# janhq/cortex.llamacpp

Measured on AMD Instinct MI355X. Metric: decode tok/s, Llama-3-8B Q4_K_M GGUF (prefill tok/s in `prefill_tok_s`), higher is better.
Workload: dtype int8 dot (Q4_K/Q6_K x Q8_K), f32 accumulate

## Files before the change

cortex.llamacpp_amd/binding.py:

```python
from __future__ import annotations

import ctypes as C
import os

import numpy as np

from .gguf_synth import (BF16, F16, F32, IQ4_NL, IQ4_XS, MXFP4, Q2_K, Q3_K, Q4_0, Q4_1, Q4_K, Q5_0, Q5_1, Q5_K, Q6_K, Q8_0, Q8_K,
                         TQ1_0, TQ2_0)

HERE = os.path.dirname(os.path.abspath(__file__))


class MI355Error(RuntimeError):
    pass


def lib_path() -> str:
    return os.environ.get("MI355_LLAMA_LIB") or os.path.join(HERE, "lib", "libmi355_llama.so")


class ModelParams(C.Structure):
    _fields_ = [("n_gpu_layers", C.c_int32), ("main_gpu", C.c_int32), ("use_mmap", C.c_int32), ("use_mlock", C.c_int32),
                ("tp_rank", C.c_int32), ("tp_size", C.c_int32), ("prefill_planes", C.c_int32)]


class ContextParams(C.Structure):
    _fields_ = [("n_ctx", C.c_uint32), ("n_batch", C.c_uint32), ("n_ubatch", C.c_uint32), ("n_seq_max", C.c_uint32),
                ("type_k", C.c_int32), ("type_v", C.c_int32), ("flash_attn", C.c_int32), ("embeddings", C.c_int32),
                ("use_graphs", C.c_int32), ("logits_to_host", C.c_int32)]


class Batch(C.Structure):
    _fields_ = [("n_tokens", C.c_int32), ("token", C.POINTER(C.c_int32)), ("embd", C.POINTER(C.c_float)),
                ("pos", C.POINTER(C.c_int32)), ("n_seq_id", C.POINTER(C.c_int32)),
                ("seq_id", C.POINTER(C.POINTER(C.c_int32))), ("logits", C.POINTER(C.c_int8))]


class PplStats(C.Structure):
    _fields_ = [("n_chunks", C.c_int64), ("count", C.c_int64), ("top1", C.c_int64), ("dead", C.c_int64), ("same_top", C.c_int64),
                ("has_base", C.c_int32), ("stopped", C.c_int32),
                ("nll", C.c_double), ("nll2", C.c_double), ("nll_base", C.c_double), ("nll2_base", C.c_double), ("kl", C.c_double), ("kl2", C.c_double)]


PPL_CALLBACK = C.CFUNCTYPE(C.c_int32, C.POINTER(PplStats), C.c_void_p)


_vp, _i32, _i64, _u32, _u64, _f32, _sz, _cp = C.c_void_p, C.c_int32, C.c_int64, C.c_uint32, C.c_uint64, C.c_float, C.c_size_t, C.c_char_p
ENGINE_CB = C.CFUNCTYPE(None, C.c_char_p, C.c_char_p, C.c_void_p)
SYMBOLS = {
    "mi355_backend_init": (C.c_int, []),
    "mi355_backend_free": (None, []),
    "mi355_device_count": (C.c_int, []),
    "mi355_last_error": (_cp, []),
    "mi355_time_us": (_i64, []),
    "mi355_print_system_info": (_cp, []),
    "mi355_model_default_params": (ModelParams, []),
    "mi355_model_load_from_file": (_vp, [_cp, ModelParams]),
    "mi355_model_free": (None, [_vp]),
    "mi355_model_n_vocab": (_i32, [_vp]),
    "mi355_model_n_embd": (_i32, [_vp]),
    "mi355_model_n_layer": (_i32, [_vp]),
    "mi355_model_n_head": (_i32, [_vp]),
    "mi355_model_n_head_kv": (_i32, [_vp]),
    "mi355_model_n_ctx_train": (_i32, [_vp]),
    "mi355_model_size": (_u64, [_vp]),
    "mi355_model_cpu_buffer": (_u64, [_vp]),
    "mi355_model_other_buffer": (_u64, [_vp]),
    "mi355_model_bytes_per_token": (_u64, [_vp]),
    "mi355_model_planes_bytes": (_u64, [_vp]),
    "mi355_debug_set_option": (C.c_int, [_cp, _i32]),
    "mi355_model_desc": (_cp, [_vp]),
    "mi355_model_meta_str": (C.c_int, [_vp, _cp, _cp, _sz]),
    "mi355_context_default_params": (ContextParams, []),
    "mi355_context_new": (_vp, [_vp, ContextParams]),
    "mi355_context_free": (None, [_vp]),
    "mi355_n_ctx": (_u32, [_vp]),
    "mi355_n_batch": (_u32, [_vp]),
    "mi355_n_ubatch": (_u32, [_vp]),
    "mi355_context_device_bytes": (_u64, [_vp]),
    "mi355_batch_init": (Batch, [_i32, _i32, _i32]),
    "mi355_batch_free": (None, [Batch]),
    "mi355_decode": (_i32, [_vp, Batch]),
    "mi355_greedy_steps": (_i32, [_vp, _i32, _i32, _i32, _i32, _vp]),
    "mi355_get_logits_ith": (C.POINTER(C.c_float), [_vp, _i32]),
    "mi355_get_argmax_ith": (_i32, [_vp, _i32]),
    "mi355_get_argmax_prob_ith": (_i32, [_vp, _i32, _vp]),
    "mi355_spec_verify": (_i32, [_vp, _i32, _vp, _vp, _vp, _vp]),
    "mi355_get_token_logprobs": (_i32, [_vp, _i32, _vp, _vp, _vp, _vp]),
    "mi355_logits_kl": (_i32, [_vp, _vp, _i32, _vp, _vp, _vp, _vp]),
    "mi355_perplexity": (_i32, [_vp, _vp, _vp, _i64, _i32, _i32, _i32, _vp, _vp, _vp, _vp, _vp]),
    "mi355_imatrix_begin": (_i32, [_vp, _i32]),
    "mi355_imatrix_end": (_i32, [_vp]),
    "mi355_imatrix_clear": (_i32, [_vp]),
    "mi355_imatrix_n_entries": (_i32, [_vp]),
    "mi355_imatrix_entry": (_i32, [_vp, _i32, _vp, _i32, _vp, _vp]),
    "mi355_imatrix_get": (_i32, [_vp, _i32, _vp, _vp]),
    "mi355_speculative_steps": (_i32, [_vp, _vp, _i32, _i32, _i32, _i32, _i32, _i32, _f32, _vp, _vp]),
    "mi355_get_topk_ith": (_i32, [_vp, _i32, _i32, _i32, _vp, _vp, _vp, _f32, _f32, _f32, _vp, _vp]),
    "mi355_debug_mega_steps": (C.c_int64, [_vp]),
    "mi355_debug_engine_steps": (C.c_int64, [_vp]),
    "mi355_debug_fused_skipped_steps": (C.c_int64, [_vp]),
    "mi355_debug_qkv_attn_launches": (C.c_int64, [_vp]),
    "mi355_debug_qkv_attn_plan": (C.c_int64, [C.c_int32] * 10 + [C.POINTER(C.c_int32)]),
    "mi355_set_embeddings": (None, [_vp, _i32]),
    "mi355_get_embeddings_ith": (C.POINTER(C.c_float), [_vp, _i32]),
    "mi355_synchronize": (None, [_vp]),
    "mi355_adapter_lora_init": (_vp, [_vp, _cp]),
    "mi355_adapter_lora_free": (None, [_vp]),
    "mi355_adapter_lora_alpha": (_f32, [_vp]),
    "mi355_adapter_lora_n_pairs": (_i32, [_vp]),
    "mi355_set_adapter_lora": (_i32, [_vp, _vp, _f32]),
    "mi355_rm_adapter_lora": (_i32, [_vp, _vp]),
    "mi355_clear_adapter_lora": (None, [_vp]),
    "mi355_op_lora_delta": (C.c_int, [_i32, _vp, _vp, _vp, _vp, _vp, _vp, _vp, _i64, _i64, _vp, _vp]),
    "mi355_kv_cache_clear": (None, [_vp]),
    "mi355_kv_cache_seq_rm": (_i32, [_vp, _i32, _i32, _i32]),
    "mi355_kv_cache_seq_cp": (None, [_vp, _i32, _i32, _i32, _i32]),
    "mi355_kv_cache_seq_add": (None, [_vp, _i32, _i32, _i32, _i32]),
    "mi355_state_seq_get_size": (_sz, [_vp, _i32]),
    "mi355_state_seq_get_data": (_sz, [_vp, _vp, _sz, _i32]),
    "mi355_state_seq_set_data": (_sz, [_vp, _vp, _sz, _i32]),
    "mi355_state_seq_save_file": (_sz, [_vp, _cp, _i32, _vp, _sz]),
    "mi355_state_seq_load_file": (_sz, [_vp, _cp, _i32, _vp, _sz, C.POINTER(C.c_size_t)]),
    "mi355_debug_state_seq_timing": (None, [_vp, _vp]),
    "mi355_kv_cache_used_cells": (_i32, [_vp]),
    "mi355_debug_enable_taps": (None, [_vp, _i32]),
    "mi355_debug_layer_out": (_i32, [_vp, _i32, _vp, _sz]),
    "mi355_op_quantize_act": (C.c_int, [_i32, _vp, _i64, _i64, _vp]),
    "mi355_op_rms_norm_quant": (C.c_int, [_vp, _vp, _i64, _i64, _f32, _vp, _vp]),
    "mi355_op_swiglu_quant": (C.c_int, [_vp, _vp, _i64, _i64, _vp]),
    "mi355_op_mul_mat": (C.c_int, [_i32, _vp, _i64, _i64, _vp, _i64, _vp, _vp, _vp]),
    "mi355_op_mul_mat_add": (C.c_int, [_i32, _vp, _i64, _i64, _vp, _i64, _vp, _vp]),
    "mi355_op_mul_mat_fused": (C.c_int, [_i32, _vp, _i64, _i64, _vp, _vp, _f32, _vp]),
    "mi355_op_mat_vec_step": (C.c_int, [_i32, _vp, _vp, _vp, _i64, _vp, _i64, _i32, _vp, _i32, _vp, _f32, _i32, _i32, _i32, _vp, _i64, _vp, _vp, _vp]),
    "mi355_op_prompt_mul_mat": (C.c_int, [_i32, _vp, _vp, _vp, _i64, _vp, _i64, _i32, _vp, _i32, _i32, _vp, _f32, _i32, _i64, _vp, _vp]),
    "mi355_op_act_q8k_planes": (C.c_int, [_i32, _vp, _vp, _vp, _f32, _i64, _i64, _vp, _vp, _vp, _vp, _vp, _vp]),
    "mi355_op_f32_to_bf16": (C.c_int, [_vp, _i64, _vp]),
    "mi355_op_mul_mat_bf16": (C.c_int, [_i32, _vp, _vp, _i64, _vp, _i64, _vp, _vp, _i32, _i32, _i32, _i32, _vp]),
    "mi355_op_ffn_gate_up": (C.c_int, [_i32, _vp, _vp, _i64, _i64, _vp, _i64, _vp]),
    "mi355_op_rms_norm_mul": (C.c_int, [_vp, _vp, _i64, _i64, _f32, _vp]),
    "mi355_op_rope": (C.c_int, [_vp, _i32, _i32, _i32, _vp, _i64, _f32, _f32, _vp, _i32]),
    "mi355_op_rope_yarn": (C.c_int, [_vp, _i32, _i32, _i32, _vp, _i64, _f32, _f32, _vp, _i32, _f32, _f32, _f32, _f32]),
    "mi355_op_get_rows": (C.c_int, [_i32, _vp, _i64, _i64, _vp, _i64, _vp]),
    "mi355_op_repack_rows": (C.c_int, [_i32, _vp, _i64, _i64, _vp]),
    "mi355_op_swiglu": (C.c_int, [_vp, _vp, _i64, _vp]),
    "mi355_op_soft_max": (C.c_int, [_vp, _vp, _i64, _i64, _f32, _vp]),
    "mi355_op_moe_route": (C.c_int, [_vp, _i64, _i32, _i32, _vp, _vp]),
    "mi355_op_moe_router": (C.c_int, [_i32, _vp, _i32, _i64, _vp, _i64, _i32, _i32, _vp, _vp, _vp, _vp]),
    "mi355_op_argmax_rows": (C.c_int, [_vp, _i64, _vp, _i32, _i32, _vp]),
    "mi355_op_argmax_prob_rows": (C.c_int, [_vp, _i64, _i32, _vp, _vp]),
    "mi355_op_spec_verify": (C.c_int, [_vp, _i64, _i32, _vp, _i32, _vp, _i32, _vp, _vp, _vp]),
    "mi355_op_token_logprob_rows": (C.c_int, [_vp, _i64, _i32, _vp, _vp, _i32, _vp, _vp]),
    "mi355_op_logits_kl_rows": (C.c_int, [_vp, _i32, _vp, _i32, _i64, _vp, _vp, _i32, _vp, _vp]),
    "mi355_op_imatrix_accum": (C.c_int, [_vp, _vp, _i64, _i64, _i32, _vp, _i32, _vp, _i32, _vp, _vp]),
    "mi355_quantize_chunk": (C.c_int, [_i32, _i32, _vp, _i64, _i64, _vp, _vp]),
    "mi355_quantize_supported": (C.c_int, [_i32]),
    "mi355_quantize_last_times": (C.c_int, [_vp, _vp, _vp]),
    "mi355_op_topk_rows": (C.c_int, [_vp, _i64, _i32, _vp, _i32, _i32, _vp, _vp, _vp, _vp, _vp, _vp, _vp, _vp]),
    "mi355_op_moe_group": (C.c_int, [_vp, _i64, _i32, _i32, _vp, _vp, _vp]),
    "mi355_op_moe_gather_act": (C.c_int, [_vp, _vp, _vp, _vp, _vp, _i64, _i64, _vp, _i64, _vp, _vp, _vp, _vp, _vp]),
    "mi355_op_moe_combine": (C.c_int, [_vp, _vp, _vp, _i64, _i32, _i32, _i32, _vp, _vp]),
    "mi355_op_moe_mul_mat_grouped": (C.c_int, [_i32, _i32, _vp, _vp, _i32, _i64, _i64, _vp, _vp, _i64, _i64, _i64, _vp, _vp]),
    "mi355_op_gather_rows_f32": (C.c_int, [_vp, _i64, _i64, _vp, _i64, _vp]),
    "mi355_op_flash_attn": (C.c_int, [_vp, _i64, _i32, _i32, _i32, _i32, _vp, _i32, _vp, _i32, _vp, _vp, _f32, _vp]),
    "mi355_op_attn_step": (C.c_int, [_vp, _vp, _vp, _i32, _i32, _i32, _i32, _vp, _i32, _vp, _i32, _vp, _i32, _i32, _f32, _i32, _f32, _i32, _vp, _i64, _vp, _i32,
                                     _vp, _vp, _vp, _vp]),
    "mi355_op_attn_decode_neox": (C.c_int, [_vp, _vp, _vp, _i32, _i32, _i32, _i32, _vp, _i32, _vp, _i32, _vp, _i32, _i32, _f32, _f32, _vp, _vp, _f32, _i32,
                                            _vp, _vp, _vp]),
    "mi355_op_flash_attn_seq": (C.c_int, [_vp, _i64, _i32, _i32, _i32, _i32, _vp, _i32, _vp, _i32, _vp, _vp, _vp, _vp, _i32, _f32, _vp]),
    "mi355_op_flash_attn_plan": (C.c_int, [_i64, _i32, _i32, _i32, _i32, _i32, _i32, _vp]),
    "mi355_op_attn_step_seq": (C.c_int, [_vp, _vp, _vp, _i32, _i32, _i32, _i32, _vp, _i32, _vp, _i32, _vp, _vp, _i32, _i32, _i32, _i32, _f32, _i32, _f32, _i32, _vp,
                                         _i64, _vp, _i32, _vp, _vp, _vp, _vp]),
    "mi355_op_attn_decode_neox_seq": (C.c_int, [_vp, _vp, _vp, _i32, _i32, _i32, _i32, _vp, _i32, _vp, _i32, _vp, _vp, _i32, _i32, _i32, _i32, _f32, _f32, _vp, _vp,
                                                _f32, _i32, _vp, _vp, _vp]),
    "mi355_op_attn_batch_step": (C.c_int, [_vp, _vp, _vp, _i64, _i32, _i32, _i32, _i32, _vp, _i32, _vp, _i32, _i32, _vp, _vp, _vp, _vp, _vp, _f32, _i32, _i32, _f32,
                                           _i32, _vp, _vp]),
    "mi355_op_attn_batch_step_planes": (C.c_int, [_vp, _vp, _vp, _i64, _i32, _i32, _i32, _i32, _vp, _i32, _vp, _i32, _i32, _vp, _vp, _vp, _vp, _vp, _f32, _i32, _i32, _f32,
                                           _i32, _vp, _vp, _vp, _vp]),
    "mi355_op_kv_store": (C.c_int, [_i32, _vp, _vp, _vp, _i64, _i32, _i32, _i32, _i32, _i32, _i32, _i32, _i32, _vp, _vp, _f32, _f32, _vp, _vp, _vp, _f32, _vp, _vp]),
    "mi355_op_k_shift": (C.c_int, [_i32, _i32, _i32, _i32, _i32, _i32, _vp, _f32, _f32, _vp, _f32, _f32, _f32, _f32, _vp]),
    "mi355_op_kv_state_pack": (C.c_int, [_i32, _i32, _i32, _i32, _i32, _i32, _vp, _vp, _vp, _i32, _vp]),
    "mi355_op_kv_state_unpack": (C.c_int, [_i32, _i32, _i32, _i32, _i32, _i32, _vp, _vp, _i32, _vp, _vp]),
    "mi355_bench_hbm_read": (C.c_double, [_sz, C.c_int]),
    "mi355_profile_last_decode": (_i32, [_vp, C.POINTER(_cp), C.POINTER(_f32), _i32]),
    "mi355_profile_enable": (None, [_vp, _i32]),
# ... 1021 lines not shown

        def as_dict(s):
            return {name: getattr(s, name) for name, _ in PplStats._fields_}

        raised = []

        def tramp(sp, _user):
            try:
                return 1 if callback(as_dict(sp.contents)) else 0
            except BaseException as ex:
                raised.append(ex)
                return 1

        cb = PPL_CALLBACK(tramp) if callback is not None else None
        r = self.lib.mi355_perplexity(self.h, base.h if base is not None else None, _ptr(tk), tk.size, n_chunk, int(bos), int(seq), _ptr(lp),
                                      _ptr(kl) if kl is not None else None, C.cast(cb, C.c_void_p) if cb is not None else None, None, C.byref(st))
        if raised:
            raise raised[0]
        if r != 0:
            raise MI355Error(f"mi355_perplexity failed: {_err(self.lib)}")
        out = as_dict(st)
        n_scored = int(st.n_chunks) * per
        out["logprobs"] = lp[:n_scored]
        if kl is not None:
            out["kls"] = kl[:n_scored]
        if st.count > 0:
            out["ppl"] = float(np.exp(st.nll / st.count))
            if base is not None:
                out["ppl_base"] = float(np.exp(st.nll_base / st.count))
                out["mean_kl"] = st.kl / st.count
        return out

    def imatrix_begin(self, process_output: bool = False) -> None:
        if self.lib.mi355_imatrix_begin(self.h, int(bool(process_output))) != 0:
            raise MI355Error(f"mi355_imatrix_begin failed: {_err(self.lib)}")

    def imatrix_end(self) -> None:
        if self.lib.mi355_imatrix_end(self.h) != 0:
            raise MI355Error(f"mi355_imatrix_end failed: {_err(self.lib)}")

    def imatrix_clear(self) -> None:
        if self.lib.mi355_imatrix_clear(self.h) != 0:
            raise MI355Error(f"mi355_imatrix_clear failed: {_err(self.lib)}")

    def imatrix_entries(self) -> dict:
        out = {}
        buf = C.create_string_buffer(256)
        for i in range(int(self.lib.mi355_imatrix_n_entries(self.h))):
            ne0, n_mat = C.c_int32(0), C.c_int32(0)
            if self.lib.mi355_imatrix_entry(self.h, i, C.cast(buf, C.c_void_p), 256, C.cast(C.byref(ne0), C.c_void_p), C.cast(C.byref(n_mat), C.c_void_p)) < 0:
                raise MI355Error(f"mi355_imatrix_entry failed: {_err(self.lib)}")
            sum2 = np.zeros((n_mat.value, ne0.value), np.float32)
            counts = np.zeros(n_mat.value, np.int32)
            if self.lib.mi355_imatrix_get(self.h, i, _ptr(sum2), _ptr(counts)) != 0:
                raise MI355Error(f"mi355_imatrix_get failed: {_err(self.lib)}")
            out[buf.value.decode()] = (sum2, counts)
        return out

    def speculative_steps(self, draft_ctx: "Context", first: int, pos0: int, n: int, n_max: int = 16, n_min: int = 0, p_min: float = 0.75, seq: int = 0):
        out = np.empty(n, np.int32); stats = np.zeros(4, np.int64)
        done = self.lib.mi355_speculative_steps(self.h, draft_ctx.h, int(first), int(pos0), int(seq), int(n), int(n_max), int(n_min), float(p_min),
                                                out.ctypes.data, stats.ctypes.data)
        if done != n:
            raise MI355Error(f"mi355_speculative_steps stopped after {done} of {n}: {_err(self.lib)}")
        return out, stats

    def mega_steps(self) -> int:
        return int(self.lib.mi355_debug_mega_steps(self.h))

    def topk(self, k: int, i: int = -1, adj_tok=(), adj_bias=(), adj_count=(), repeat: float = 1.0, freq: float = 0.0, present: float = 0.0):
        at = np.ascontiguousarray(adj_tok, np.int32); ab = np.ascontiguousarray(adj_bias, np.float32); ac = np.ascontiguousarray(adj_count, np.int32)
        toks = np.zeros(k, np.int32); lg = np.zeros(k, np.float32)
        r = self.lib.mi355_get_topk_ith(self.h, i, k, at.size, _ptr(at), _ptr(ab), _ptr(ac), repeat, freq, present, _ptr(toks), _ptr(lg))
        if r != k:
            raise MI355Error(f"mi355_get_topk_ith failed: {_err(self.lib)}")
        return toks, lg

    def fused_skipped_steps(self) -> int:
        return int(self.lib.mi355_debug_fused_skipped_steps(self.h))

    def qkv_attn_launches(self) -> int:
        return int(self.lib.mi355_debug_qkv_attn_launches(self.h))

    def engine_steps(self) -> int:
        return int(self.lib.mi355_debug_engine_steps(self.h))

    def synchronize(self):
        self.lib.mi355_synchronize(self.h)

    def kv_clear(self):
        self.lib.mi355_kv_cache_clear(self.h)

    def kv_seq_rm(self, seq, p0, p1) -> bool:
        return bool(self.lib.mi355_kv_cache_seq_rm(self.h, seq, p0, p1))

    def kv_seq_cp(self, s, d, p0, p1):
        self.lib.mi355_kv_cache_seq_cp(self.h, s, d, p0, p1)

    def kv_seq_add(self, seq, p0, p1, delta):
        self.lib.mi355_kv_cache_seq_add(self.h, seq, p0, p1, delta)

    def state_seq_size(self, seq: int = 0) -> int:
        return int(self.lib.mi355_state_seq_get_size(self.h, int(seq)))

    def state_seq_get(self, seq: int = 0) -> bytes:
        buf = np.zeros(self.state_seq_size(seq), np.uint8)
        n = int(self.lib.mi355_state_seq_get_data(self.h, _ptr(buf), buf.size, int(seq)))
        if n == 0:
            raise MI355Error(f"mi355_state_seq_get_data refused: {_err(self.lib)}")
        return buf[:n].tobytes()

    def state_seq_set(self, seq: int, blob) -> int:
        buf = np.frombuffer(bytes(blob), np.uint8)
        n = int(self.lib.mi355_state_seq_set_data(self.h, buf.ctypes.data if buf.size else None, buf.size, int(seq)))
        if n == 0:
            raise MI355Error(f"mi355_state_seq_set_data refused: {_err(self.lib)}")
        return n

    def state_seq_save_file(self, path: str, seq: int, tokens) -> int:
        tokens = np.ascontiguousarray(tokens, np.int32).reshape(-1)
        n = int(self.lib.mi355_state_seq_save_file(self.h, os.fsencode(path), int(seq), _ptr(tokens), tokens.size))
        if n == 0:
            raise MI355Error(f"mi355_state_seq_save_file refused: {_err(self.lib)}")
        return n

    def state_seq_load_file(self, path: str, seq: int, max_tokens: int = 1 << 20) -> np.ndarray:
        toks = np.zeros(max_tokens, np.int32)
        n_tok = C.c_size_t(0)
        n = int(self.lib.mi355_state_seq_load_file(self.h, os.fsencode(path), int(seq), _ptr(toks), toks.size, C.byref(n_tok)))
        if n == 0:
            raise MI355Error(f"mi355_state_seq_load_file refused: {_err(self.lib)}")
        return toks[:n_tok.value].copy()

    def state_seq_timing(self):
        out = np.zeros(3, np.float32)
        self.lib.mi355_debug_state_seq_timing(self.h, _ptr(out))
        return tuple(float(x) for x in out)

    def kv_used(self) -> int:
        return int(self.lib.mi355_kv_cache_used_cells(self.h))

    def enable_taps(self, on: bool = True):
        self.lib.mi355_debug_enable_taps(self.h, int(on))

    def layer_out(self, il: int, n_tokens: int) -> np.ndarray:
        out = np.zeros((n_tokens, self.model.n_embd), np.float32)
        n = self.lib.mi355_debug_layer_out(self.h, il, _ptr(out), out.size)
        if n < 0:
            raise MI355Error("debug taps not enabled")
        return out[:n]

    def profile(self, on: bool = True):
        self.lib.mi355_profile_enable(self.h, int(on))

    def last_profile(self) -> dict:
        names = (_cp * 64)()
        us = (_f32 * 64)()
        n = self.lib.mi355_profile_last_decode(self.h, names, us, 64)
        return {names[i].decode(): float(us[i]) for i in range(n)}

    def force_moe_ids(self, ids: np.ndarray) -> None:
        ids = np.ascontiguousarray(ids, np.int32)
        rc = self.lib.mi355_debug_force_moe_ids(self.h, _ptr(ids), ids.shape[0], ids.shape[1], ids.shape[2])
        if rc != 0:
            raise MI355Error(f"mi355_debug_force_moe_ids failed ({rc}): {_err(self.lib)}")

# ... 89 lines not shown
```

cortex.llamacpp_amd/csrc/c_api.cc:

```cpp
#include "../../include/mi355_llama.h"

#include <atomic>
#include <memory>
#include <new>
#include <chrono>
#include <cmath>
#include <cstdio>
#include <cstdlib>
#include <cstring>
#include <string>
#include <vector>

#include "../host/clip.h"
#include "../host/engine.h"
#include "../host/hip_backend.h"
#include "../host/log.h"
#include "../host/runtime.h"
#include "../host/attn_chunks.h"
#include "../host/tp_comm.h"
#include "../host/tp_split.h"
#include "../host/vocab.h"

namespace mi355 {
const std::string &last_error_string();
// ... 332 lines not shown
        if (stats) memcpy(stats, st, sizeof st);
        int32_t sid = seq;
        int32_t *sp = &sid;
        int32_t n_seq[SPEC_MAX_DRAFT + 2], pos[SPEC_MAX_DRAFT + 2], toks[SPEC_MAX_DRAFT + 2], ids[SPEC_MAX_DRAFT + 1], draft[SPEC_MAX_DRAFT + 1];
        int32_t *seqs[SPEC_MAX_DRAFT + 2];
        int8_t flags[SPEC_MAX_DRAFT + 2];
        for (int j = 0; j < SPEC_MAX_DRAFT + 2; j++) { n_seq[j] = 1; seqs[j] = sp; }
        auto decode = [&](Context *c, int cnt, bool all_rows) -> bool {
            for (int j = 0; j < cnt; j++) flags[j] = all_rows || j == cnt - 1;
            const int rc = c->decode(cnt, toks, pos, n_seq, seqs, flags);
            if (rc != 0) fail(rc < 0 ? c->last_error : std::string("speculative_steps: no KV cells left for the batch"));
            return rc == 0;
        };
        const int room = (int)std::min(T->cp.n_ctx / T->cp.n_seq_max, D->cp.n_ctx / D->cp.n_seq_max);
        std::vector<int32_t> pend;
        int32_t last = first, p = pos0, dpos = pos0, done = 0;
        while (done < n) {
            const int k_cap = std::max(0, std::min((int)n_max, room - p - 1));
            int k = 0;
            pend.push_back(last);
            if (k_cap > 0) {
                if (pend.size() > (size_t)SPEC_MAX_DRAFT + 2) { fail("speculative_steps: the draft context fell behind"); break; }
                for (size_t j = 0; j < pend.size(); j++) { toks[j] = pend[j]; pos[j] = dpos + (int32_t)j; }
                if (!decode(D, (int)pend.size(), false)) break;
                dpos = p + 1;
                pend.clear();
                bool bad = false;
                for (;;) {
                    float pr = 0.0f;
                    const int32_t t = D->argmax_prob_ith(-1, &pr);
                    if (t < 0) { fail(D->last_error); bad = true; break; }
                    if (pr < p_min) break;
                    draft[k++] = t;
                    if (k == k_cap) break;
                    toks[0] = t; pos[0] = dpos;
                    if (!decode(D, 1, false)) { bad = true; break; }
                    dpos++;
                }
                if (bad) break;
                if (k < n_min) k = 0;
            }
            int a = 0;
            toks[0] = last; pos[0] = p;
            for (int j = 0; j < k; j++) { toks[j + 1] = draft[j]; pos[j + 1] = p + 1 + j; }
            if (!decode(T, k + 1, true)) break;
            if (k > 0) {
                const int32_t gs[2] = {0, k + 1};
                draft[k] = -1;
                if (T->spec_verify(1, gs, draft, ids, &a) < 0) { fail(T->last_error); break; }
            } else {
                ids[0] = T->argmax_ith(0);
                if (ids[0] < 0) { fail(T->last_error.empty() ? "arg-max failed" : T->last_error); break; }
                st[3]++;
            }
            const int m = std::min(a + 1, (int)(n - done));
            st[0]++; st[1] += k; st[2] += m - 1;
            for (int j = 0; j < m; j++) if (out_tokens) out_tokens[done + j] = ids[j];
            done += m;
            const int32_t keep = p + m;
            if (k + 1 > m) T->kv_seq_rm(seq, keep, -1);
            if (dpos > keep) { D->kv_seq_rm(seq, keep, -1); dpos = keep; }
            for (int32_t q = dpos + (int32_t)pend.size(); q < keep; q++) pend.push_back(q == p ? last : ids[q - p - 1]);
            last = ids[m - 1];
            p = keep;
        }
        if (stats) memcpy(stats, st, sizeof st);
        return done;
    )
}
int32_t mi355_get_topk_ith(mi355_context *ctx, int32_t i, int32_t k, int32_t n_adj, const int32_t *adj_tok, const float *adj_bias, const int32_t *adj_count,
                           float penalty_repeat, float penalty_freq, float penalty_present, int32_t *toks_out, float *logits_out) {
    if (!ctx || !toks_out || !logits_out || n_adj < 0 || n_adj > TOPK_MAX_ADJ || (n_adj > 0 && (!adj_tok || !adj_bias || !adj_count))) { fail("bad arguments"); return -1; }
    TopkAdj a{};
    a.n = n_adj; a.repeat = penalty_repeat; a.freq = penalty_freq; a.present = penalty_present;
    for (int j = 0; j < n_adj; j++) { a.tok[j] = adj_tok[j]; a.bias[j] = adj_bias[j]; a.cnt[j] = adj_count[j]; }
    const int r = ctx->c->topk_ith(i, k, a, toks_out, logits_out);
    if (r < 0) fail(ctx->c->last_error.empty() ? "top-k failed" : ctx->c->last_error);
    return r;
}
int64_t mi355_debug_mega_steps(const mi355_context *ctx) { return ctx->c->mega_steps; }
int64_t mi355_debug_engine_steps(const mi355_context *ctx) { return ctx->c->engine_steps; }
int64_t mi355_debug_fused_skipped_steps(const mi355_context *ctx) { return ctx->c->fused_skipped_steps; }
int64_t mi355_debug_qkv_attn_launches(const mi355_context *ctx) { return ctx->c->qkv_attn_launches; }
int64_t mi355_debug_qkv_attn_plan(int32_t type_q, int32_t type_k, int32_t type_v, int32_t type_o, int32_t n_embd, int32_t n_head, int32_t n_head_kv, int32_t head_dim,
                                  int32_t type_kv, int32_t n_kv, int32_t *slots_out) {
    int slots = 0;
    const size_t lds = qkv_attn_out_plan_lds(type_q, type_k, type_v, type_o, n_embd, n_head, n_head_kv, head_dim, type_kv, n_kv, &slots);
    if (slots_out) *slots_out = slots;
    return (int64_t)lds;
}
void mi355_set_embeddings(mi355_context *ctx, int32_t enabled) { ctx->c->embeddings_enabled = enabled != 0 || ctx->c->model->hp.encoder; }
float *mi355_get_embeddings_ith(mi355_context *ctx, int32_t i) { return ctx->c->embeddings_ith(i); }
void mi355_synchronize(mi355_context *ctx) { ctx->c->synchronize(); }

mi355_adapter_lora *mi355_adapter_lora_init(mi355_model *model, const char *path) {
    if (!model || !path) { fail("null model or path"); return nullptr; }
    MI355_GUARD(return nullptr,
        std::string err;
        int status = 0;
        LoraAdapter *a = lora_load(model->m, path, err, status);
        if (!a) { fail(err); return nullptr; }
        mi355_adapter_lora *h = new (std::nothrow) mi355_adapter_lora;
        if (!h) { lora_free(a); fail("out of host memory"); return nullptr; }
        h->a = a;
        return h;
    )
}
void mi355_adapter_lora_free(mi355_adapter_lora *adapter) {
    if (!adapter) return;
    lora_free(adapter->a);
    delete adapter;
}
float mi355_adapter_lora_alpha(const mi355_adapter_lora *adapter) { return adapter ? adapter->a->alpha : 0.0f; }
int32_t mi355_adapter_lora_n_pairs(const mi355_adapter_lora *adapter) { return adapter ? (int32_t)adapter->a->pairs.size() : 0; }
int32_t mi355_set_adapter_lora(mi355_context *ctx, mi355_adapter_lora *adapter, float scale) {
    if (!ctx || !adapter) { fail("null context or adapter"); return MI355_ERR_ARG; }
    MI355_GUARD(return MI355_ERR_ARG,
        if (ctx->c->set_adapter_lora(adapter->a, scale) != 0) { fail(ctx->c->last_error); return MI355_ERR_ARG; }
        return MI355_OK;
    )
}
int32_t mi355_rm_adapter_lora(mi355_context *ctx, mi355_adapter_lora *adapter) {
    if (!ctx || !adapter) { fail("null context or adapter"); return MI355_ERR_ARG; }
    if (ctx->c->rm_adapter_lora(adapter->a) != 0) { fail(ctx->c->last_error); return -1; }
    return MI355_OK;
}
void mi355_clear_adapter_lora(mi355_context *ctx) { if (ctx) ctx->c->clear_adapter_lora(); }

mi355_clip *mi355_clip_model_load(const char *path, int32_t main_gpu) {
    if (!path) { fail("clip_model_load: no path"); return nullptr; }
    MI355_GUARD(return nullptr,
        std::unique_ptr<mi355_clip> c(new mi355_clip);
        const std::string err = c->m.load(path, main_gpu < 0 ? 0 : main_gpu);
        if (!err.empty()) { fail(err); return nullptr; }
        return c.release();
    )
}
void mi355_clip_free(mi355_clip *clip) { delete clip; }
int32_t mi355_clip_n_mmproj_embd(const mi355_clip *clip) { return clip ? clip->m.proj_dim : 0; }
int32_t mi355_clip_n_patches(const mi355_clip *clip) { return clip ? clip->m.n_patches() : 0; }
int32_t mi355_clip_image_size(const mi355_clip *clip) { return clip ? clip->m.image_size : 0; }
int32_t mi355_clip_max_image_rows(const mi355_clip *clip) { return clip ? clip->m.max_image_rows() : 0; }
int32_t mi355_clip_image_preprocess_grid(const mi355_clip *clip, const uint8_t *rgb, int32_t nx, int32_t ny, float *out, size_t out_floats, int32_t *grid_w, int32_t *grid_h) {
    if (!clip || !rgb || !out || nx <= 0 || ny <= 0) { fail("clip_image_preprocess_grid: bad arguments"); return MI355_ERR_ARG; }
    MI355_GUARD(return MI355_ERR_ARG,
        ClipImageU8 img;
        img.nx = nx; img.ny = ny; img.rgb.assign(rgb, rgb + (size_t)3 * nx * ny);
        std::vector<std::vector<float>> imgs;
        int gw = 0, gh = 0;
        clip->m.preprocess_all(img, imgs, gw, gh);
        const size_t per = (size_t)3 * clip->m.image_size * clip->m.image_size;
        if (out_floats < per * imgs.size()) { fail("clip_image_preprocess_grid: output buffer too small"); return MI355_ERR_ARG; }
        for (size_t i = 0; i < imgs.size(); i++) memcpy(out + i * per, imgs[i].data(), per * sizeof(float));
        if (grid_w) *grid_w = gw;
        if (grid_h) *grid_h = gh;
        return (int32_t)imgs.size();
    )
}
int32_t mi355_clip_image_load_from_bytes(const uint8_t *bytes, size_t n_bytes, int32_t *nx, int32_t *ny, uint8_t *rgb_out, size_t rgb_cap) {
    MI355_GUARD(return MI355_ERR_ARG,
        ClipImageU8 img;
        const std::string err = clip_image_load_from_bytes(bytes, n_bytes, img);
        if (!err.empty()) { fail(err); return MI355_ERR_ARG; }
        if (nx) *nx = img.nx;
        if (ny) *ny = img.ny;
        if (rgb_out) {
// ... 1820 lines not shown
    std::vector<KVLayerView> views;
    std::unique_ptr<DevBuf> table, cells, rows;
    size_t row_bytes = 0;
    int init(int type_k, int type_v, int n_layer, int G, int D, int n_cells, const void *const *k_rows, const void *const *v_rows, const int32_t *cell_list, int n, bool distinct) {
        if (!k_rows || !v_rows || !cell_list || n_layer < 1 || n_layer > 1024 || G < 1 || D < 32 || D % 32 || n_cells < 1 || n < 1 || n > n_cells) { fail("kv_state: bad geometry / null argument"); return MI355_ERR_ARG; }
        if ((type_k != T_F16 && type_k != T_Q8_0 && type_k != T_Q4_0) || (type_v != T_F16 && type_v != T_Q8_0 && type_v != T_Q4_0)) { fail("kv_state: bad cache type"); return MI355_ERR_ARG; }
        std::vector<char> seen((size_t)n_cells, 0);
        for (int i = 0; i < n; i++) {
            if (cell_list[i] < 0 || cell_list[i] >= n_cells) { fail("kv_state: cells[" + std::to_string(i) + "] outside the cache"); return MI355_ERR_ARG; }
            if (distinct && seen[(size_t)cell_list[i]]) { fail("kv_state: cells[" + std::to_string(i) + "] listed twice"); return MI355_ERR_ARG; }
            seen[(size_t)cell_list[i]] = 1;
        }
        views.resize((size_t)n_layer);
        for (int il = 0; il < n_layer; il++) {
            if (!k_rows[il] || !v_rows[il]) { fail("kv_state: null layer"); return MI355_ERR_ARG; }
            std::vector<uint8_t> kc, vc;
            std::vector<uint16_t> ks, vs;
            cache_planes_from_rows(type_k, k_rows[il], G, D, n_cells, kc, ks);
            cache_planes_from_rows(type_v, v_rows[il], G, D, n_cells, vc, vs);
            DevBuf *b[4] = {new DevBuf(kc.size()), new DevBuf(ks.size() * 2 + 16), new DevBuf(vc.size()), new DevBuf(vs.size() * 2 + 16)};
            for (DevBuf *p : b) bufs.emplace_back(p);
            if (!b[0]->up(kc.data(), kc.size()) || !b[2]->up(vc.data(), vc.size()) || !b[1]->p || !b[3]->p || (!ks.empty() && !b[1]->up(ks.data(), ks.size() * 2)) ||
                (!vs.empty() && !b[3]->up(vs.data(), vs.size() * 2))) { fail("device alloc/copy failed"); return MI355_ERR_OOM; }
            views[(size_t)il].k = b[0]->as<uint8_t>(); views[(size_t)il].kd = b[1]->as<uint16_t>(); views[(size_t)il].v = b[2]->as<uint8_t>(); views[(size_t)il].vd = b[3]->as<uint16_t>();
        }
        row_bytes = (size_t)n_layer * n * (kv_state_row_bytes(type_k, G, D) + kv_state_row_bytes(type_v, G, D));
        table.reset(new DevBuf(views.size() * sizeof(KVLayerView)));
        cells.reset(new DevBuf((size_t)n * 4));
        rows.reset(new DevBuf(row_bytes));
        if (!table->up(views.data(), views.size() * sizeof(KVLayerView)) || !cells->up(cell_list, (size_t)n * 4) || !rows->p) { fail("device alloc/copy failed"); return MI355_ERR_OOM; }
        return MI355_OK;
    }
};
}

int mi355_op_kv_state_pack(int32_t type_k, int32_t type_v, int32_t n_layer, int32_t G, int32_t D, int32_t n_cells, const void *const *k_rows, const void *const *v_rows,
                           const int32_t *cells, int32_t n, void *out) {
    if (!need_device()) return MI355_ERR_NO_DEVICE;
    if (!out) { fail("kv_state_pack: null output"); return MI355_ERR_ARG; }
    StateOpCache c;
    if (const int rc = c.init(type_k, type_v, n_layer, G, D, n_cells, k_rows, v_rows, cells, n, false)) return rc;
    hipError_t e = launch_kv_state_pack(c.table->as<KVLayerView>(), n_layer, type_k, type_v, G, D, n_cells, c.cells->as<int32_t>(), n, c.rows->as<uint8_t>(), nullptr);
    if (e == hipSuccess) e = hipDeviceSynchronize();
    if (e != hipSuccess) return hip_fail(e, "kv_state_pack");
    return c.rows->down(out, c.row_bytes) ? MI355_OK : MI355_ERR_HIP;
}

int mi355_op_kv_state_unpack(int32_t type_k, int32_t type_v, int32_t n_layer, int32_t G, int32_t D, int32_t n_cells, const void *in, const int32_t *cells, int32_t n,
                             void *const *k_rows, void *const *v_rows) {
    if (!need_device()) return MI355_ERR_NO_DEVICE;
    if (!in) { fail("kv_state_unpack: null input"); return MI355_ERR_ARG; }
    StateOpCache c;
    if (const int rc = c.init(type_k, type_v, n_layer, G, D, n_cells, k_rows, v_rows, cells, n, true)) return rc;
    if (!c.rows->up(in, c.row_bytes)) { fail("device alloc/copy failed"); return MI355_ERR_OOM; }
    hipError_t e = launch_kv_state_unpack(c.table->as<KVLayerView>(), n_layer, type_k, type_v, G, D, n_cells, c.cells->as<int32_t>(), n, c.rows->as<uint8_t>(), nullptr);
    if (e == hipSuccess) e = hipDeviceSynchronize();
    if (e != hipSuccess) return hip_fail(e, "kv_state_unpack");
    for (int il = 0; il < n_layer; il++)
        if (!cache_rows_from_planes(type_k, *c.bufs[(size_t)il * 4], *c.bufs[(size_t)il * 4 + 1], G, D, n_cells, k_rows[il]) ||
            !cache_rows_from_planes(type_v, *c.bufs[(size_t)il * 4 + 2], *c.bufs[(size_t)il * 4 + 3], G, D, n_cells, v_rows[il])) return MI355_ERR_HIP;
    return MI355_OK;
}

int mi355_debug_set_option(const char *name, int32_t value) {
    if (!name) return MI355_ERR_ARG;
    if (!strcmp(name, "mmq_planes")) { g_op_mmq_planes = value != 0; return MI355_OK; }
    if (!strcmp(name, "mmq_tiles")) { mmq_set_tiles(value); return MI355_OK; }
    if (!strcmp(name, "mmq_q80_tiles")) { mmq_q80_set_tiles(value); return MI355_OK; }
    if (!strcmp(name, "mmq_split")) { mmq_set_split(value); return MI355_OK; }
    if (!strcmp(name, "mmq_lds_form")) { mmq_set_lds_form(value); return MI355_OK; }
    if (!strcmp(name, "mmq_ksplit")) { g_op_mmq_ksplit = value != 0; return MI355_OK; }
    if (!strcmp(name, "attn_store_fuse")) { set_attn_store_fuse(value != 0); return MI355_OK; }
    if (!strcmp(name, "rope_fast")) { set_rope_fast(value != 0); return MI355_OK; }
    if (!strcmp(name, "decode_mega") || !strcmp(name, "decode_engine")) {
        if (value > 0 && !experiments_built()) { fail(std::string(name) + ": the experiment kernels are not in this build (MI355_BUILD_EXPERIMENTS=1 python cortex.llamacpp_amd/build.py --force)"); return MI355_ERR_ARG; }
        if (name[7] == 'm') set_decode_mega(value != 0); else set_decode_engine(value);
        return MI355_OK;
    }
    if (!strcmp(name, "tp_p2p")) { tp_p2p_use(value != 0); return MI355_OK; }
    if (!strcmp(name, "tp_p2p_prompt")) { tp_p2p_use_prompt(value != 0); return MI355_OK; }
    if (!strcmp(name, "mmvq_stream")) { mmvq_set_stream(value != 0); return MI355_OK; }
    if (!strcmp(name, "attn_out_fused")) { set_attn_out_fused(value); return MI355_OK; }
    if (!strcmp(name, "qkv_attn_fused")) { set_qkv_attn_fused(value); return MI355_OK; }
    if (!strcmp(name, "moe_group_min")) { set_moe_group_min(value); return MI355_OK; }
    if (!strcmp(name, "moe_q80_grouped")) { set_moe_q80_grouped(value != 0); return MI355_OK; }
    if (!strcmp(name, "fa_v_acc_f16")) { set_fa_v_acc_f16(value); return MI355_OK; }
    if (!strcmp(name, "raise_stream_error")) { debug_raise_stream_error((unsigned)value); return MI355_OK; }
    if (!strcmp(name, "state_stage_kib")) { set_state_stage_max((size_t)(value > 0 ? value : 0) * 1024); return MI355_OK; }
    if (!strcmp(name, "tp_null_group")) { tp_set_null_group(0, value); return MI355_OK; }
    fail(std::string("unknown option ") + name);
    return MI355_ERR_ARG;
}

int mi355_tp_unique_id(void *id_out, size_t cap) {
    if (!need_device()) return MI355_ERR_NO_DEVICE;
    std::string err;
    const int n = tp_unique_id(id_out, cap, err);
    if (n < 0) { fail(err); return MI355_ERR_ARG; }
    return n;
}
int mi355_tp_init(int32_t device, int32_t rank, int32_t size, const void *id, size_t id_len) {
    if (!need_device()) return MI355_ERR_NO_DEVICE;
    if (hipSetDevice(device) != hipSuccess) { fail("hipSetDevice failed"); return MI355_ERR_ARG; }
    std::string err;
    if (tp_init(rank, size, id, id_len, err) != 0) { fail(err); return MI355_ERR_ARG; }
    return MI355_OK;
}
void mi355_tp_shutdown(void) { tp_shutdown(); }
int mi355_tp_worker_main(int sock_fd) {
    try {
        if (!g_backend_ok && mi355_backend_init() != MI355_OK) return 66;
        return tp_split_worker_main(sock_fd);
    } catch (const std::exception &e) {
        fprintf(stderr, "mi355_tp_worker: %s\n", e.what());
        return 70;
    } catch (...) { return 70; }
}
int32_t mi355_tp_rank(void) { return tp_rank(); }
int32_t mi355_tp_size(void) { return tp_size(); }
int mi355_tp_set_host_exchange(mi355_tp_host_exchange fn, void *user, int32_t rank, int32_t size) {
    if (fn && (size < 1 || rank < 0 || rank >= size)) { fail("bad rank / size"); return MI355_ERR_ARG; }
    tp_set_host_exchange(reinterpret_cast<tp_host_exchange_fn>(fn), user, rank, size);
    return MI355_OK;
}

int mi355_tp_p2p_local_handle2(void *out, size_t cap, size_t max_floats, size_t prompt_floats) {
    if (!need_device()) return MI355_ERR_NO_DEVICE;
    std::string err;
    const int n = tp_p2p_local_handle(out, cap, max_floats, prompt_floats, err);
    if (n < 0) { fail(err); return MI355_ERR_ARG; }
    return n;
}
int mi355_tp_p2p_local_handle(void *out, size_t cap, size_t max_floats) { return mi355_tp_p2p_local_handle2(out, cap, max_floats, 0); }
int mi355_tp_p2p_enable(const void *handles, size_t len) {
    if (!need_device()) return MI355_ERR_NO_DEVICE;
    std::string err;
    if (tp_p2p_enable(handles, len, err) != 0) { fail(err); return MI355_ERR_HIP; }
    return MI355_OK;
}
int64_t mi355_tp_p2p_exchanges(void) { return tp_p2p_exchanges(); }
int64_t mi355_tp_p2p_prompt_exchanges(void) { return tp_p2p_prompt_exchanges(); }

double mi355_bench_hbm_read(size_t bytes, int iters) {
    if (!need_device()) return -1.0;
    return hbm_read_probe(bytes, iters);
}

static Vocab *model_vocab(mi355_model *m) {
    if (!m) { fail("null model"); return nullptr; }
    if (!m->vocab_tried) {
        m->vocab_tried = true;
        std::string err;
        m->vocab_ok = m->vocab.load(*m->m->file, err);
        if (!m->vocab_ok) fail("tokenizer: " + err);
    }
    return m->vocab_ok ? &m->vocab : nullptr;
}
int32_t mi355_tokenize(mi355_model *m, const char *text, int32_t text_len, mi355_token *out, int32_t cap, int32_t add_special, int32_t parse_special) {
    MI355_GUARD(return INT32_MIN,
        Vocab *v = model_vocab(m);
        if (!v || !text || text_len < 0) return INT32_MIN;
        const std::vector<int32_t> ids = v->tokenize(std::string(text, (size_t)text_len), add_special != 0, parse_special != 0);
        if ((int64_t)ids.size() > cap || !out) return -(int32_t)ids.size();
        memcpy(out, ids.data(), ids.size() * sizeof(int32_t));
        return (int32_t)ids.size();
    )
// ... 108 lines not shown
```

cortex.llamacpp_amd/host/runtime.cc:

```cpp
#include "runtime.h"

#include <dlfcn.h>
#include "tp_comm.h"
#include "attn_chunks.h"

#include <algorithm>
#include <atomic>
#include <cmath>
#include <cstdarg>
#include <cstdio>
#include <cstring>

namespace mi355 {

unsigned stream_error_epoch();
static unsigned *stream_error_word();

static thread_local std::string g_err;
void set_error(const char *fmt, ...) {
    char buf[1024];
    va_list ap;
    va_start(ap, fmt);
    vsnprintf(buf, sizeof buf, fmt, ap);
    va_end(ap);
// ... 1116 lines not shown
        return launch_mmf16(w.data, (int)w.N, K, x_f32, T, out, ld_out, epi == EPI_ADD ? resid : nullptr, stream_);
    return launch_mmv_float(w.type, w.data, (int)w.N, K, x_f32, T, out, ld_out, epi == EPI_ADD ? resid : nullptr, stream_);
}

static bool bf16_takes_mfma(const DevTensor *const *ws, float *const *outs, int n, int K, int T, int ld_out, const void *xb) {
    bool mfma = true;
    for (int i = 0; i < n; i++) mfma &= mmbf16_applicable(T_BF16, (int)ws[i]->N, K, T, ws[i]->data, xb, outs[i]) && ws[i]->n_expert == 1 && ((n == 1 ? ld_out : (int)ws[i]->N) & 3) == 0;
    return mfma;
}

hipError_t Context::linear_bf16(const DevTensor *const *ws, float *const *outs, const float *const *bias, int n, int K, int T, int ld_out, const float *resid, int epi) {
    if (bf16_takes_mfma(ws, outs, n, K, T, ld_out, xb_)) {
        for (int i = 0; i < n; i++)
            HIP_TRY(launch_mmbf16(ws[i]->data, (int)ws[i]->N, K, xb_, T, outs[i], n == 1 ? ld_out : (int)ws[i]->N, epi == EPI_ADD ? resid : nullptr, bias ? bias[i] : nullptr, 1.0f, false, stream_));
        if (epi == EPI_SWIGLU) HIP_TRY(launch_swiglu(outs[0], outs[1], outs[0], (int64_t)T * ws[0]->N, stream_));
        return hipSuccess;
    }
    MMVBF16Args a{};
    a.n_seg = n; a.K = K; a.epi = epi; a.resid = epi == EPI_ADD ? resid : nullptr; a.xb = xb_;
    for (int i = 0; i < n; i++) a.seg[i] = MMVBF16Seg{ws[i]->data, outs[i], bias ? bias[i] : nullptr, (int)ws[i]->N, n == 1 ? ld_out : (int)ws[i]->N, ws[i]->row_bytes};
    return launch_mmv_bf16_tokens(a, T, stream_);
}

hipError_t Context::linear_multi(const DevTensor *const *ws, float *const *outs, int n, const ActQuant &aq, const float *x_f32, int T, const float *const *bias, bool *bias_done) {
    bool all_q = true, all_bf = n <= 3;
    for (int i = 0; i < n; i++) { all_q &= type_is_quant(ws[i]->type); all_bf &= ws[i]->type == T_BF16 && ws[i]->n_expert == 1; }
    const int K = (int)ws[0]->K;
    if (all_bf) {
        HIP_TRY(launch_f32_to_bf16(x_f32, xb_, (size_t)T * K, stream_));
        HIP_TRY(linear_bf16(ws, outs, bias, n, K, T, 0, nullptr, EPI_STORE));
        if (bias_done) *bias_done = true;
        return hipSuccess;
    }
    const PromptMatmul pm = pending_fuse_.mode == 0 ? prompt_mul_mat_choice(PM_ROLE_MULTI, ws, n, K, T, mmq_ws_) : PromptMatmul();
    if (pm.form == PM_KSPLIT) {
        HIP_TRY(ensure_prep(aq, K, T));
        MMQSeg sg[3];
        for (int i = 0; i < n; i++) sg[i] = MMQSeg{ws[i]->data, ws[i]->row_bytes, (int)ws[i]->N, ws[i]->type, outs[i], (int)ws[i]->N, nullptr, 0};
        return launch_mmq_ksplit_multi(sg, n, K, T, aq, mmq_bh_, mmq_bl_, false, stream_);
    }
    if (pm.form == PM_PLANES) {
        HIP_TRY(ensure_prep(aq, K, T));
        const int nf = pm.n_fused;
        if (nf >= 2) {
            int rows[3], ldo[3], types[3];
            float *o[3];
            for (int i = 0; i < nf; i++) { rows[i] = (int)ws[i]->N; ldo[i] = (int)ws[i]->N; o[i] = outs[i]; types[i] = ws[i]->type; }
            HIP_TRY(launch_mmq_planes_multi(ws[0]->type, ws[0]->planes, rows, o, ldo, nf, K, T, aq, mmq_bh_, mmq_bl_, nullptr, stream_, mmq_ws_, types));
        }
        for (int i = nf; i < n; i++) {
            if (ws[i]->planes) HIP_TRY(launch_mmq_planes(ws[i]->type, ws[i]->planes, (int)ws[i]->N, K, T, aq, mmq_bh_, mmq_bl_, outs[i], (int)ws[i]->N, nullptr, stream_, mmq_ws_));
            else HIP_TRY(launch_mmq(ws[i]->type, ws[i]->data, ws[i]->row_bytes, (int)ws[i]->N, K, T, aq, mmq_bh_, mmq_bl_, outs[i], (int)ws[i]->N, nullptr, stream_));
        }
        return hipSuccess;
    }
    bool any_mmq = false;
    for (int i = 0; i < n; i++) any_mmq |= mmq_applicable(ws[i]->type, K, T) || mmq_q80_applicable(ws[i]->type, K, T) || planes_small(*ws[i], K, T) || q80_copy(*ws[i], K, T);
    if (all_q && n <= 3 && !(any_mmq && pending_fuse_.mode == 0)) {
        MMVQSeg segs[3];
        for (int i = 0; i < n; i++) segs[i] = make_seg(*ws[i], outs[i], (int)ws[i]->N, nullptr, nullptr);
        return mmvq_tokens(segs, n, K, T, EPI_STORE, aq, stream_, pending_fuse_);
    }
    for (int i = 0; i < n; i++) {
        hipError_t e = linear(*ws[i], aq, x_f32, K, T, outs[i], (int)ws[i]->N, nullptr, EPI_STORE);
        if (e != hipSuccess) return e;
    }
    return hipSuccess;
}

static int g_moe_group_min = getenv("MI355_MOE_GROUP_MIN") ? atoi(getenv("MI355_MOE_GROUP_MIN")) : 8;
void set_moe_group_min(int t) { g_moe_group_min = t < 1 ? 1 : t; }
static bool g_moe_q80_grouped = !(getenv("MI355_MOE_Q80_GROUPED") && getenv("MI355_MOE_Q80_GROUPED")[0] == '0');
void set_moe_q80_grouped(bool on) { g_moe_q80_grouped = on; }
static int g_decode_mega = -1;
static bool g_store_fuse = true;
void set_attn_store_fuse(bool on) { g_store_fuse = on; }
static bool store_fuse_enabled() {
    static const bool env_off = getenv("MI355_ATTN_STORE_FUSE") && getenv("MI355_ATTN_STORE_FUSE")[0] == '0';
    return g_store_fuse && !env_off;
}
static bool g_rope_fast = true;
void set_rope_fast(bool on) { g_rope_fast = on; }
void set_decode_mega(bool on) { g_decode_mega = on ? 1 : 0; }

bool Context::mega_prepare() {
    if (mega_state_ != 0) return mega_state_ > 0;
    mega_state_ = -1;
    static const bool mega_env_on = getenv("MI355_MEGA") && getenv("MI355_MEGA")[0] == '1';
    const bool mega_env = g_decode_mega < 0 ? mega_env_on : g_decode_mega > 0;
    const HParams &hp = model->hp;
    const int E = hp.n_embd, FF = hp.n_ff, H = hp.n_head, G = hp.n_head_kv, D = hp.head_dim;
    if (!mega_env || hp.n_expert > 0 || G <= 0 || H % G != 0 || H * D != E) return false;
    const int kb_e = (E + 2047) >> 11, kb_ff = (FF + 2047) >> 11;
    if ((E % 2048) != 0 || (FF % 256) != 0 || !decode_mega_applicable(kb_e, kb_ff, H / G, cp.type_k, cp.type_v, hp.qk_norm)) return false;
    RopeArgs ra = rope_args(*model, false);
    if (ra.neox || (ra.n_rot % 4) != 0 || D != 128 || !kv_store_fast_applicable(G, D, cp.type_k, cp.type_v, ra)) return false;
    std::vector<MegaLayer> ml((size_t)hp.n_layer);
    const int blocks = mega_blocks();
    size_t lds = 0;
    for (int il = 0; il < hp.n_layer; il++) {
        const LayerWeights &L = model->layers[(size_t)il];
        if (!type_is_kq456(L.wq.type) || !type_is_kq456(L.wk.type) || !type_is_kq456(L.wv.type) || !type_is_kq456(L.wo.type) || !type_is_kq456(L.gate.type) || !type_is_kq456(L.up.type) || !type_is_kq456(L.down.type)) return false;
        if (L.gate.type != L.up.type || L.gate.N != L.up.N || L.bq.valid() || L.bk.valid() || L.bv.valid()) return false;
        if ((int)L.wq.K != E || (int)L.wo.K != E || (int)L.gate.K != E || (int)L.down.K != FF) return false;
        MegaLayer &m = ml[(size_t)il];
        m.qkv = single_token_desc(3, E, EPI_STORE, 1, x_, (const float *)L.attn_norm.data, hp.eps, aq_e_);
        m.qkv.seg[0] = make_seg(L.wq, q_, (int)L.wq.N, nullptr, nullptr);
        m.qkv.seg[1] = make_seg(L.wk, k_, (int)L.wk.N, nullptr, nullptr);
        m.qkv.seg[2] = make_seg(L.wv, v_, (int)L.wv.N, nullptr, nullptr);
        m.wo = single_token_desc(1, E, EPI_ADD, 0, nullptr, nullptr, hp.eps, aq_o_);
        m.wo.seg[0] = make_seg(L.wo, x_, E, x_, nullptr);
        m.gate_up = single_token_desc(2, E, EPI_SWIGLU, 1, x_, (const float *)L.ffn_norm.data, hp.eps, aq_e_);
        m.gate_up.seg[0] = make_seg(L.gate, ffn_, FF, nullptr, nullptr);
        m.gate_up.seg[1] = make_seg(L.up, ffn_u_, FF, nullptr, nullptr);
        m.down = single_token_desc(1, FF, EPI_ADD, 2, ffn_, nullptr, hp.eps, aq_ff_);
        m.down.seg[0] = make_seg(L.down, x_, E, x_, nullptr);
        for (MMVQArgs *a : {&m.qkv, &m.wo, &m.gate_up, &m.down}) {
            if (!mmvq_fast_applicable(*a)) return false;
            const size_t l = mmvq_fast_plan(*a, blocks, 4);
            if (!l) return false;
            lds = std::max(lds, l);
        }
        m.kv = kv_[(size_t)il];
    }
    d_mega_layers_ = (MegaLayer *)dalloc(ml.size() * sizeof(MegaLayer));
    if (hipExtMallocWithFlags((void **)&d_mega_sync_, MEGA_SYNC_WORDS * sizeof(unsigned), hipDeviceMallocUncached) != hipSuccess) { d_mega_sync_ = nullptr; return false; }
    allocs_.push_back(d_mega_sync_);
    if (!d_mega_layers_ || !d_mega_sync_) return false;
    if (!h_mega_flag_ && hipHostMalloc((void **)&h_mega_flag_, sizeof(int), hipHostMallocDefault) != hipSuccess) return false;
    *h_mega_flag_ = 0;
    if (hipMemcpy(d_mega_layers_, ml.data(), ml.size() * sizeof(MegaLayer), hipMemcpyHostToDevice) != hipSuccess) return false;
    if (hipMemset(d_mega_sync_, 0, MEGA_SYNC_WORDS * sizeof(unsigned)) != hipSuccess || hipDeviceSynchronize() != hipSuccess) return false;
    if (getenv("MI355_MEGA_PROBE") && getenv("MI355_MEGA_PROBE")[0] == '1')
        d_mega_probe_ = (unsigned long long *)dalloc((size_t)(1 + MEGA_PROBES_PER_LAYER * hp.n_layer) * 8);
    mega_lds_ = lds;
    mega_state_ = 1;
    return true;
}

bool Context::mega_check() {
    if (mega_state_ <= 0 || !h_mega_flag_ || *h_mega_flag_ == 0) return true;
    *h_mega_flag_ = 0;
    (void)hipMemset(d_mega_sync_, 0, MEGA_SYNC_WORDS * sizeof(unsigned));
    (void)hipDeviceSynchronize();
    mega_state_ = -1;
    for (auto &ge : graphs_) (void)hipGraphExecDestroy(ge.second);
    graphs_.clear();
    graph_exec_ = nullptr;
    last_error = "whole-step kernel: device-wide barrier timed out (workgroups not co-resident?); results of the step discarded";
    return false;
}

static int g_decode_engine = -1;
void set_decode_engine(int on) { g_decode_engine = on < 0 ? -1 : on ? 1 : 0; }

static unsigned *stream_error_word() {
    static unsigned *w = [] { unsigned *p = nullptr; if (hipHostMalloc((void **)&p, 64, hipHostMallocDefault) != hipSuccess) p = nullptr; if (p) *p = 0u; return p; }();
    return w;
}

unsigned *install_stream_error_word() {
    unsigned *ew = stream_error_word();
    if (ew) { mmvq_stream_set_error_word(ew); decode_engine_set_error_word(ew); attn_out_set_error_word(ew); tp_p2p_set_error_word(ew); }
    return ew;
}

// ... 91 lines not shown
    if (hipMemcpy(d_engine_layers_, el.data(), el.size() * sizeof(EngineLayer), hipMemcpyHostToDevice) != hipSuccess) return false;
    if (hipMemset(d_engine_gran_, 0, gw * 8) != hipSuccess || hipDeviceSynchronize() != hipSuccess) return false;
    if (const char *pl = getenv("MI355_ENGINE_PROBE")) {
        engine_probe_layer_ = atoi(pl);
        const size_t np = (size_t)num_cu() * 10 * 48;
        d_engine_probe_ = (unsigned long long *)dalloc(np * 8);
        if (d_engine_probe_) (void)hipMemset(d_engine_probe_, 0, np * 8);
        (void)hipDeviceSynchronize();
    }
    engine_state_ = 1;
    return true;
}

hipError_t Context::run_layers_encoder(int T, int n_kv_cap) {
    cur_T_ = T;
    const HParams &hp = model->hp;
    const int E = hp.n_embd, FF = hp.n_ff, H = hp.n_head, G = hp.n_head_kv, D = hp.head_dim;
    RopeArgs ra = rope_args(*model, true);
    const int n_kv_max = std::max(n_kv_cap, 1);
    att_splits_ = flash_attn_pick_splits(T, G, n_kv_max);
    last_layers_mega_ = false; last_layers_engine_ = false;
    HIP_TRY(launch_step_setup_embed(d_pos_, T, ra, rope_cs_, d_cell_pos_, d_cell_seq_, d_cell_, d_seqmask_, nullptr, nullptr, model->tok_embd.type, model->tok_embd.data, E,
                                    d_tok_, x_, stream_));
    if (model->tok_types.valid())
        HIP_TRY(launch_add_qkv_bias(x_, nullptr, nullptr, (const float *)model->tok_types.data, nullptr, nullptr, E, 0, T, stream_));
    HIP_TRY(launch_layer_norm(x_, (const float *)model->tok_norm.data, (const float *)model->tok_norm_b.data, E, T, hp.eps, x_, stream_));
    prof_mark("embed");
    auto quantise_for = [&](const float *x, int K, ActQuant &aq, std::initializer_list<const DevTensor *> ws) -> hipError_t {
        bool k = false, z = false;
        for (const DevTensor *w : ws) if (type_is_quant(w->type)) { if (act_is_q80(w->type)) z = true; else k = true; }
        if (!k && !z) return hipSuccess;
        prep_owner_ = nullptr;
        return launch_quantize(x, K, T, aq, k, z, stream_);
    };
    for (int il = 0; il < hp.n_layer; il++) {
        const LayerWeights &L = model->layers[(size_t)il];
        HIP_TRY(quantise_for(x_, E, aq_e_, {&L.wq, &L.wk, &L.wv}));
        const DevTensor *ws[3] = {&L.wq, &L.wk, &L.wv};
        float *outs[3] = {q_, k_, v_};
        HIP_TRY(linear_multi(ws, outs, 3, aq_e_, x_, T));
        prof_mark("qkv");
        HIP_TRY(launch_rope_kv_store(q_, k_, v_, T, H, G, D, d_pos_, d_cell_, ra, kv_[(size_t)il], cp.type_k, cp.type_v, (int)cp.n_ctx, rope_cs_, stream_));
        prof_mark("rope_kv");
        AttnArgs aa = attn_args(il, T, n_kv_max, d_pos_open_);
        aa.splits = att_splits_;
        aa.pf_splits = flash_attn_prefill_splits(T, H, G, D, n_kv_max);
        while (aa.pf_splits > 1 && flash_attn_workspace_floats(T, H, D, aa.pf_splits) > att_part_floats_) aa.pf_splits >>= 1;
        HIP_TRY(launch_flash_attn(aa, stream_));
        prof_mark("attn");
        HIP_TRY(quantise_for(att_, H * D, aq_o_, {&L.wo}));
        HIP_TRY(linear(L.wo, aq_o_, att_, H * D, T, q_, E, nullptr, EPI_STORE));
        if (L.bo.valid()) HIP_TRY(launch_add_qkv_bias(q_, nullptr, nullptr, (const float *)L.bo.data, nullptr, nullptr, E, 0, T, stream_));
        HIP_TRY(launch_add(q_, x_, xn_, (int64_t)T * E, stream_));
        HIP_TRY(launch_layer_norm(xn_, (const float *)L.attn_out_norm.data, (const float *)L.attn_out_norm_b.data, E, T, hp.eps, xn_, stream_));
        prof_mark("attn_out");
        HIP_TRY(quantise_for(xn_, E, aq_e_, {&L.gate, &L.up}));
        HIP_TRY(linear(L.gate, aq_e_, xn_, E, T, ffn_, FF, nullptr, EPI_STORE));
        HIP_TRY(linear(L.up, aq_e_, xn_, E, T, ffn_u_, FF, nullptr, EPI_STORE));
        HIP_TRY(launch_swiglu(ffn_, ffn_u_, ffn_, (int64_t)T * FF, stream_));
        prof_mark("ffn_gate_up");
        HIP_TRY(quantise_for(ffn_, FF, aq_ff_, {&L.down}));
        HIP_TRY(linear(L.down, aq_ff_, ffn_, FF, T, q_, E, nullptr, EPI_STORE));
        HIP_TRY(launch_add(q_, xn_, x_, (int64_t)T * E, stream_));
        HIP_TRY(launch_layer_norm(x_, (const float *)L.layer_out_norm.data, (const float *)L.layer_out_norm_b.data, E, T, hp.eps, x_, stream_));
        prof_mark("ffn_down");
        if (debug_taps_ && dbg_) HIP_TRY(hipMemcpyAsync(dbg_ + (size_t)il * cp.n_ubatch * E, x_, (size_t)T * E * 4, hipMemcpyDeviceToDevice, stream_));
    }
    return hipSuccess;
}


Context::Step Context::step_constants(int T, int n_kv_cap) const {
    static const int attn_mode = getenv("MI355_ATTN_MODE") ? atoi(getenv("MI355_ATTN_MODE")) : 2;
    static const bool rope_fast_env = !(getenv("MI355_ROPE_FAST") && getenv("MI355_ROPE_FAST")[0] == '0');
    static const bool fuse_down_env = !(getenv("MI355_FUSE_DOWN") && getenv("MI355_FUSE_DOWN")[0] == '0');
    const HParams &hp = model->hp;
    Step st;
    st.T = T;
    st.n_kv_max = std::max(n_kv_cap, 1);
    st.ra_step = rope_args(*model, true);
    st.tp = hp.tp_exchange;
    st.chunk_lists = chunk_lmax_ > 0;
    st.attn_mode = attn_mode; st.rope_fast = rope_fast_env && g_rope_fast; st.fuse_down_env = fuse_down_env;
    st.out = st.tp ? tp_part_ : x_;
    st.resid = !st.tp || hp.tp_rank == 0 ? x_ : nullptr;
    return st;
}

AttnArgs Context::attn_args(int il, int T, int n_kv_max, const int32_t *tok_pos) const {
    const HParams &hp = model->hp;
    AttnArgs aa{};
    aa.q = q_; aa.out = att_; aa.kv = kv_[(size_t)il]; aa.type_k = cp.type_k; aa.type_v = cp.type_v;
    aa.T = T; aa.H = hp.n_head; aa.G = hp.n_head_kv; aa.D = hp.head_dim; aa.n_ctx = (int)cp.n_ctx;
    aa.cell_pos = d_cell_pos_; aa.cell_seq = d_cell_seq_; aa.tok_pos = tok_pos; aa.tok_seq = d_seq_;
    aa.n_kv_dev = d_nkv_; aa.n_kv_max = n_kv_max; aa.scale = 1.0f / sqrtf((float)hp.head_dim); aa.part = att_part_;
    return aa;
}
void Context::attn_chunk_lists(AttnArgs &aa) const {
    aa.tok_chunks = d_chunks_; aa.tok_nchunks = d_chunks_ + (size_t)64 * chunk_stride_; aa.chunk_stride = chunk_stride_;
    aa.splits = std::max(chunk_cap_, chunk_lmax_);
}

Context::AttnPlan Context::plan_attn(int il, const Step &st) const {
    const HParams &hp = model->hp;
    const LayerWeights &L = model->layers[(size_t)il];
    const int E = hp.n_embd, T = st.T;
    AttnPlan p{};
    p.ra = layer_rope(st.ra_step, L, hp.eps);
    p.qkv_float = !type_is_quant(L.wq.type) || !type_is_quant(L.wk.type) || !type_is_quant(L.wv.type);
    p.qkv_lora = f32_rows(il, LORA_Q) || f32_rows(il, LORA_K) || f32_rows(il, LORA_V);
    p.qkv_prologue = !p.qkv_float && can_fuse(E, T) && !p.qkv_lora;
    AttnArgs &aa = p.aa;
    aa = attn_args(il, T, st.n_kv_max, d_pos_);
    const bool o_q = type_is_quant(L.wo.type);
    aa.out_q = o_q ? &aq_o_ : nullptr; aa.out_q8k = !act_is_q80(L.wo.type); aa.out_q80 = act_is_q80(L.wo.type);
    p.o_planes = o_q && aa.out_q8k && T >= 3;
    if (p.o_planes) { aa.out_bh = mmq_bh_; aa.out_bl = mmq_bl_; }
    const bool v16 = fa_v_acc_f16_enabled() && cp.type_k == T_F16 && cp.type_v == T_F16;
    p.decode_attn = !v16 && flash_attn_decode_applicable(aa, p.ra);
    if (p.decode_attn) {
        aa.splits = flash_attn_decode_splits(st.n_kv_max);
        if (st.chunk_lists) attn_chunk_lists(aa);
        p.fused_step = st.attn_mode > 0 && flash_attn_decode_fused_applicable(aa, p.ra);
    }
    p.ao_seg = make_seg(L.wo, st.out, E, st.resid, nullptr);
    p.ao_epi = st.resid ? EPI_ADD : EPI_STORE;
    p.af = aa;
    if (p.decode_attn && p.fused_step && st.attn_mode == 2 && !st.engine && il < 255 && !attn_out_off_ && !attn_out_skip_step_ && !(st.tp && tp_uses_host()) && !f32_rows(il, LORA_O)) {
        p.af.splits = attn_out_fused_splits(p.af);
        if (st.chunk_lists) p.af.splits = aa.splits;
        p.ao_form = attn_out_fused_applicable(p.af, p.ra, p.ao_seg, (int)L.wo.K, p.ao_epi);
    }
    if (p.ao_form && p.qkv_prologue && !st.tp && d_qkv_gran_ && !(L.bq.valid() || L.bk.valid() || L.bv.valid())) {
        QKVFuse &qf = p.qf;
        qf.seg[0] = make_seg(L.wq, q_, (int)L.wq.N, nullptr, nullptr);
        qf.seg[1] = make_seg(L.wk, k_, (int)L.wk.N, nullptr, nullptr);
        qf.seg[2] = make_seg(L.wv, v_, (int)L.wv.N, nullptr, nullptr);
        qf.nx = x_; qf.nw = (const float *)L.attn_norm.data; qf.neps = hp.eps; qf.K = E; qf.gran = d_qkv_gran_;
        p.qkv_in_attn = qkv_attn_out_applicable(p.af, p.ra, p.ao_seg, (int)L.wo.K, p.ao_epi, qf);
    }
    return p;
}

hipError_t Context::attn_qkv(int il, const Step &st, const AttnPlan &p) {
    const HParams &hp = model->hp;
    const LayerWeights &L = model->layers[(size_t)il];
    const int E = hp.n_embd, T = st.T;
    if (p.qkv_in_attn) return hipSuccess;
    if (st.engine && il > 0) return hipSuccess;
    if (p.qkv_prologue) {
        pending_fuse_.mode = 1; pending_fuse_.x = x_; pending_fuse_.w = (const float *)L.attn_norm.data; pending_fuse_.eps = hp.eps;
    } else {
        const bool need_k = (type_is_quant(L.wq.type) && !act_is_q80(L.wq.type)) || (type_is_quant(L.wk.type) && !act_is_q80(L.wk.type)) || (type_is_quant(L.wv.type) && !act_is_q80(L.wv.type));
        const bool need_0 = act_is_q80(L.wq.type) || act_is_q80(L.wk.type) || act_is_q80(L.wv.type);
        const bool pl = need_k && T >= 3;
        HIP_TRY(launch_rmsnorm_quant(x_, (const float *)L.attn_norm.data, E, T, hp.eps, p.qkv_float || p.qkv_lora ? xn_ : nullptr, &aq_e_, need_k, need_0, stream_,
                                     pl ? mmq_bh_ : nullptr, pl ? mmq_bl_ : nullptr));
        prep_owner_ = nullptr;
        if (pl) prep_written(aq_e_, E, T);
        prof_mark("norm_quant");
        if (imx_on_) HIP_TRY(imx_collect(il, IMX_QKV, xn_, nullptr, E, T, nullptr, nullptr));
    }
    const DevTensor *ws[3] = {&L.wq, &L.wk, &L.wv};
    float *outs[3] = {q_, k_, v_};
    const float *bias[3] = {L.bq.valid() ? (const float *)L.bq.data : nullptr, L.bk.valid() ? (const float *)L.bk.data : nullptr, L.bv.valid() ? (const float *)L.bv.data : nullptr};
    bool bias_done = false;
    HIP_TRY(linear_multi(ws, outs, 3, aq_e_, xn_, T, bias, &bias_done));
    pending_fuse_ = Fuse();
    if (p.qkv_lora) {
        const int targets[3] = {LORA_Q, LORA_K, LORA_V}, lds[3] = {(int)L.wq.N, (int)L.wk.N, (int)L.wv.N};
        HIP_TRY(lora_add(il, targets, outs, lds, 3, xn_, E, E, T));
    }
    if (!bias_done && (bias[0] || bias[1] || bias[2]))
        HIP_TRY(launch_add_qkv_bias(q_, k_, v_, bias[0], bias[1], bias[2], hp.n_head * hp.head_dim, hp.n_head_kv * hp.head_dim, T, stream_));
    prof_mark("qkv");
    return hipSuccess;
}

hipError_t Context::attn_core(int il, const Step &st, const AttnPlan &p) {
    const HParams &hp = model->hp;
    const LayerWeights &L = model->layers[(size_t)il];
    const int H = hp.n_head, G = hp.n_head_kv, D = hp.head_dim, T = st.T;
    const KVLayerView &kv = kv_[(size_t)il];
    unsigned *ao_flags = d_ao_flags_ + (size_t)il * 64 * ATT_SYNC_STRIDE;
    if (p.qkv_in_attn) {
        HIP_TRY(launch_qkv_attn_out(p.af, rope_cs_, p.ra, d_cell_, att_counters_, ao_flags, d_ao_gran_, il, d_step_serial_, p.ao_seg, (int)L.wo.K, p.ao_epi, p.qf, stream_));
        qkv_attn_launches++;
        prof_mark("qkv");
    } else if (p.fused_step) {
        if (p.ao_form)
            HIP_TRY(launch_attn_out_fused(p.af, rope_cs_, p.ra, k_, v_, d_cell_, att_counters_, ao_flags, d_ao_gran_, il, d_step_serial_, p.ao_seg, (int)L.wo.K, p.ao_epi, stream_));
        else
            HIP_TRY(launch_flash_attn_decode_fused(p.aa, rope_cs_, p.ra, k_, v_, d_cell_, st.attn_mode == 2 ? att_counters_ : nullptr, stream_));
    } else if (p.decode_attn && batch_distinct_ && store_fuse_enabled()) {
        HIP_TRY(launch_flash_attn_decode(p.aa, rope_cs_, p.ra, stream_, k_, v_, d_cell_));
    } else if (p.decode_attn && kv_store_fast_applicable(G, D, cp.type_k, cp.type_v, p.ra)) {
        HIP_TRY(launch_kv_store_fast(k_, v_, T, G, D, rope_cs_, p.ra, d_cell_, kv, cp.type_k, cp.type_v, (int)cp.n_ctx, stream_));
        prof_mark("rope_kv");
        HIP_TRY(launch_flash_attn_decode(p.aa, rope_cs_, p.ra, stream_));
    } else {
        if (st.rope_fast && rope_cs_ && rope_q_kv_store_fast_applicable(H, G, D, cp.type_k, cp.type_v, p.ra))
            HIP_TRY(launch_rope_q_kv_store_fast(q_, k_, v_, T, H, G, D, rope_cs_, p.ra, d_cell_, kv, cp.type_k, cp.type_v, (int)cp.n_ctx, stream_));
        else
            HIP_TRY(launch_rope_kv_store(q_, k_, v_, T, H, G, D, d_pos_, d_cell_, p.ra, kv, cp.type_k, cp.type_v, (int)cp.n_ctx, rope_cs_, stream_));
        prof_mark("rope_kv");
        AttnArgs aa = p.aa;
        aa.splits = att_splits_;
        aa.pf_splits = flash_attn_prefill_splits(T, H, G, D, std::min(st.n_kv_max, cur_max_pos_ + 1));
        while (aa.pf_splits > 1 && flash_attn_workspace_floats(T, H, D, aa.pf_splits) > att_part_floats_) aa.pf_splits >>= 1;
        HIP_TRY(launch_flash_attn(aa, stream_));
    }
    prof_mark("attn");
    if (p.o_planes) prep_written(aq_o_, (int)L.wo.K, T);
    else if (prep_owner_ == aq_o_.qs) prep_owner_ = nullptr;
    return hipSuccess;
}

hipError_t Context::attn_output(int il, const Step &st, const AttnPlan &p) {
    const LayerWeights &L = model->layers[(size_t)il];
    if (p.ao_form) return hipSuccess;
    HIP_TRY(linear(L.wo, aq_o_, att_, (int)L.wo.K, st.T, st.out, model->hp.n_embd, st.resid, p.ao_epi));
    if (imx_on_) HIP_TRY(imx_collect(il, IMX_O, att_, nullptr, (int)L.wo.K, st.T, nullptr, nullptr));
    if (lora_on(il, LORA_O)) {
        const int target = LORA_O, ld = model->hp.n_embd;
        float *out = st.out;
        HIP_TRY(lora_add(il, &target, &out, &ld, 1, att_, (int)L.wo.K, (int)L.wo.K, st.T));
    }
    return hipSuccess;
}

hipError_t Context::quantise_for_down(int il, int T, bool combined, bool planes_any_T) {
    const int FF = model->hp.n_ff;
    const bool k = !act_is_q80(model->layers[(size_t)il].down.type), pl = k && (planes_any_T || T >= 3);
    int8_t *bh = pl ? mmq_bh_ : nullptr, *bl = pl ? mmq_bl_ : nullptr;
    if (combined) HIP_TRY(launch_quantize(ffn_, FF, T, aq_ff_, k, !k, stream_, bh, bl));
    else HIP_TRY(launch_swiglu_quant(ffn_, ffn_u_, FF, T, aq_ff_, k, !k, stream_, bh, bl));
    prep_owner_ = nullptr;
    if (pl) prep_written(aq_ff_, FF, T);
    return hipSuccess;
}

hipError_t Context::ffn_dense_gate_up(int il, const Step &st, bool &quantised) {
    const HParams &hp = model->hp;
    const LayerWeights &L = model->layers[(size_t)il];
    const int E = hp.n_embd, FF = hp.n_ff, T = st.T;
    quantised = false;
    const bool gq = type_is_quant(L.gate.type), uq = type_is_quant(L.up.type);
    const bool fk = (gq && !act_is_q80(L.gate.type)) || (uq && !act_is_q80(L.up.type));
    const bool f0 = act_is_q80(L.gate.type) || act_is_q80(L.up.type);
    const bool lora_gu = f32_rows(il, LORA_GATE) || f32_rows(il, LORA_UP), lora_any = lora_gu || f32_rows(il, LORA_DOWN);
    const bool fuse_ffn = gq && uq && L.gate.type == L.up.type && can_fuse(E, T) && !lora_any;
    Fuse fz;
    if (fuse_ffn) {
        fz.mode = 1; fz.x = x_; fz.w = (const float *)L.ffn_norm.data; fz.eps = hp.eps;
    } else {
        const bool pl = fk && T >= 3;
        HIP_TRY(launch_rmsnorm_quant(x_, (const float *)L.ffn_norm.data, E, T, hp.eps, (!gq || !uq || lora_gu) ? xn_ : nullptr, &aq_e_, fk, f0, stream_,
                                     pl ? mmq_bh_ : nullptr, pl ? mmq_bl_ : nullptr));
        prep_owner_ = nullptr;
        if (pl) prep_written(aq_e_, E, T);
        prof_mark("norm_quant");
        if (imx_on_) HIP_TRY(imx_collect(il, IMX_FFN_IN, xn_, nullptr, E, T, nullptr, nullptr));
    }
    const bool down_q = type_is_quant(L.down.type) && (FF % 32) == 0;
    const bool ffn_mmq = (mmq_q80_applicable(L.gate.type, E, T) && mmq_q80_applicable(L.up.type, E, T)) ||
                         (mmq_applicable(L.gate.type, E, T) && mmq_applicable(L.up.type, E, T)) ||
                         (mmq_ksplit_applicable(L.gate.type, E, T) && mmq_ksplit_applicable(L.up.type, E, T)) ||
                         (planes_small(L.gate, E, T) && planes_small(L.up, E, T)) || (q80_copy(L.gate, E, T) && q80_copy(L.up, E, T));
    const DevTensor *gu_w[2] = {&L.gate, &L.up};
    const PromptMatmul gu_pm = fuse_ffn ? PromptMatmul() : prompt_mul_mat_choice(PM_ROLE_GATE_UP, gu_w, 2, E, T, mmq_ws_);
    const bool ffn_ks = gu_pm.form == PM_KSPLIT;
    if (lora_any) {
        HIP_TRY(linear(L.gate, aq_e_, xn_, E, T, ffn_, FF, nullptr, EPI_STORE));
        HIP_TRY(linear(L.up, aq_e_, xn_, E, T, ffn_u_, FF, nullptr, EPI_STORE));
        if (lora_gu) {
            const int targets[2] = {LORA_GATE, LORA_UP}, lds[2] = {FF, FF};
            float *outs[2] = {ffn_, ffn_u_};
            HIP_TRY(lora_add(il, targets, outs, lds, 2, xn_, E, E, T));
        }
        quantised = T > 1 && down_q && !f32_rows(il, LORA_DOWN);
        if (quantised) HIP_TRY(quantise_for_down(il, T, false, false));
        else HIP_TRY(launch_swiglu(ffn_, ffn_u_, ffn_, (int64_t)T * FF, stream_));
        if (imx_on_) HIP_TRY(imx_collect(il, IMX_FFN_DOWN, ffn_, nullptr, FF, T, nullptr, nullptr));
    } else if (gq && uq && L.gate.type == L.up.type && !ffn_mmq) {
        MMVQSeg segs[2] = {make_seg(L.gate, ffn_, FF, nullptr, nullptr), make_seg(L.up, ffn_u_, FF, nullptr, nullptr)};
        HIP_TRY(mmvq_tokens(segs, 2, E, T, EPI_SWIGLU, aq_e_, stream_, fz));
    } else if (L.gate.type == T_BF16 && L.up.type == T_BF16 && L.gate.N == L.up.N) {
        const DevTensor *gu[2] = {&L.gate, &L.up};
        float *go[2] = {ffn_, ffn_u_};
        HIP_TRY(launch_f32_to_bf16(xn_, xb_, (size_t)T * E, stream_));
        quantised = T > 1 && down_q && bf16_takes_mfma(gu, go, 2, E, T, 0, xb_);
        HIP_TRY(linear_bf16(gu, go, nullptr, 2, E, T, 0, nullptr, quantised ? EPI_STORE : EPI_SWIGLU));
        if (quantised) HIP_TRY(quantise_for_down(il, T, false, false));
    } else if (ffn_ks) {
        if (gu_pm.need_prep) HIP_TRY(ensure_prep(aq_e_, E, T));
        MMQSeg sg[2] = {{L.gate.data, L.gate.row_bytes, (int)L.gate.N, L.gate.type, ffn_, FF, nullptr, 0},
                        {L.up.data, L.up.row_bytes, (int)L.up.N, L.up.type, ffn_u_, FF, nullptr, 0}};
        const bool pair = gu_pm.swiglu;
        HIP_TRY(launch_mmq_ksplit_multi(sg, 2, E, T, aq_e_, mmq_bh_, mmq_bl_, pair, stream_));
        quantised = !pair && down_q;
        if (quantised) HIP_TRY(quantise_for_down(il, T, false, true));
        else if (!pair) HIP_TRY(launch_swiglu(ffn_, ffn_u_, ffn_, (int64_t)T * FF, stream_));
    } else if (T > 1 && gu_pm.form == PM_PLANES) {
        HIP_TRY(launch_mmq_planes_swiglu(L.gate.type, L.gate.planes, L.up.planes, (int)L.gate.N, E, T, aq_e_, ffn_, FF, stream_));
        quantised = down_q;
        if (quantised) HIP_TRY(quantise_for_down(il, T, true, false));
    } else {
        HIP_TRY(linear(L.gate, aq_e_, xn_, E, T, ffn_, FF, nullptr, EPI_STORE));
        HIP_TRY(linear(L.up, aq_e_, xn_, E, T, ffn_u_, FF, nullptr, EPI_STORE));
        quantised = T > 1 && down_q;
        if (quantised) HIP_TRY(quantise_for_down(il, T, false, false));
        else HIP_TRY(launch_swiglu(ffn_, ffn_u_, ffn_, (int64_t)T * FF, stream_));
    }
    prof_mark("ffn_gate_up");
    return hipSuccess;
}

hipError_t Context::ffn_down(int il, const Step &st, bool quantised, int *n_matvec) {
    const HParams &hp = model->hp;
    const LayerWeights &L = model->layers[(size_t)il];
    const int E = hp.n_embd, FF = hp.n_ff, T = st.T;
    const int epi = st.resid ? EPI_ADD : EPI_STORE;
    const bool lora_down = f32_rows(il, LORA_DOWN);
    const bool fuse_down = !lora_down && st.fuse_down_env && T == 1 && type_is_quant(L.down.type) &&
                           (((FF % 256) == 0 && mmvq_fast_kb_ok((FF + 2047) / 2048)) || ((FF % 256) != 0 && (FF % 32) == 0 && FF <= 8192 && act_is_q80(L.down.type)));
    if (fuse_down && !st.tp && L.down_lo.valid() && L.down_hi.valid()) {
        const int Kh = (int)L.down_lo.K;
        pending_fuse_.mode = 2; pending_fuse_.x = ffn_;
        HIP_TRY(linear(L.down_lo, aq_ff_, ffn_, Kh, T, st.out, E, st.resid, epi));
        pending_fuse_.mode = 2; pending_fuse_.x = ffn_ + Kh;
        HIP_TRY(linear(L.down_hi, aq_ff_, ffn_ + Kh, Kh, T, st.out, E, st.out, EPI_ADD));
        pending_fuse_ = Fuse();
        if (n_matvec) *n_matvec = 2;
        return hipSuccess;
    }
    if (n_matvec) *n_matvec = 1;
    if (fuse_down) {
        pending_fuse_.mode = 2; pending_fuse_.x = ffn_;
    } else if (type_is_quant(L.down.type) && !quantised) {
        HIP_TRY(launch_quantize(ffn_, FF, T, aq_ff_, !act_is_q80(L.down.type), act_is_q80(L.down.type), stream_));
        prep_owner_ = nullptr;
        prof_mark("quant");
    }
    HIP_TRY(linear(L.down, aq_ff_, ffn_, FF, T, st.out, E, st.resid, epi));
    pending_fuse_ = Fuse();
    if (lora_down) {
        const int target = LORA_DOWN;
        float *out = st.out;
        HIP_TRY(lora_add(il, &target, &out, &E, 1, ffn_, FF, FF, T));
    }
    return hipSuccess;
}

bool Context::moe_selected_desc(int il, MMVQArgs &a, MMVQArgs &d) const {
    const HParams &hp = model->hp;
    const LayerWeights &L = model->layers[(size_t)il];
    const int E = hp.n_embd, FF = hp.n_ff, KU = hp.n_expert_used;
    if (KU < 2 || KU > 8 || (int)cp.n_ubatch < KU || L.gate_exps.type != L.up_exps.type) return false;
    const bool prologue = can_fuse(E, 1) && !act_is_q80(L.gate_exps.type);
    a = single_token_desc(2, E, EPI_SWIGLU, prologue ? 1 : 0, prologue ? x_ : nullptr, prologue ? (const float *)L.ffn_norm.data : nullptr, prologue ? hp.eps : 0.0f, aq_e_);
    a.n_sel = KU; a.sel_out_stride = FF;
    a.seg[0] = make_seg(L.gate_exps, ffn_, FF, nullptr, moe_ids_);
    a.seg[1] = make_seg(L.up_exps, ffn_u_, FF, nullptr, moe_ids_);
    d = single_token_desc(1, FF, EPI_STORE, 2, ffn_, nullptr, 0.0f, aq_ff_);
    d.n_sel = KU; d.sel_nx_stride = FF; d.sel_out_stride = E;
    d.seg[0] = make_seg(L.down_exps, moe_out_, E, nullptr, moe_ids_);
    return mmvq_fast_applicable(a) && mmvq_fast_applicable(d);
}

hipError_t Context::moe_grouped_one_launch(int il, int T) {
    const HParams &hp = model->hp;
    const LayerWeights &L = model->layers[(size_t)il];
    const int E = hp.n_embd, FF = hp.n_ff, KU = hp.n_expert_used, NE = hp.n_expert, GR = T * KU;
    HIP_TRY(launch_moe_gather_act(aq_e_, moe_tok_, GR, E, aq_eg_, stream_));
    prep_owner_ = nullptr;
    const size_t ps_gu = L.gate_exps.planes_bytes / (size_t)L.gate_exps.n_expert, ps_d = L.down_exps.planes_bytes / (size_t)L.down_exps.n_expert;
    HIP_TRY(launch_mmq_planes_swiglu_moe(L.gate_exps.type, L.gate_exps.planes, L.up_exps.planes, ps_gu, NE, moe_meta_, (int)L.gate_exps.N, E, GR, aq_eg_, ffn_g_, FF, stream_));
    if (imx_on_) HIP_TRY(imx_collect(il, IMX_FFN_DOWN, ffn_g_, nullptr, FF, GR, nullptr, moe_meta_));
    HIP_TRY(launch_quantize(ffn_g_, FF, GR, aq_ffg_, true, false, stream_));
    HIP_TRY(launch_mmq_planes_moe(L.down_exps.type, L.down_exps.planes, ps_d, NE, moe_meta_, (int)L.down_exps.N, FF, GR, aq_ffg_, y_g_, E, stream_));
    return launch_moe_scatter_combine(x_, y_g_, moe_w_, moe_slot_, T, E, KU, stream_);
}

hipError_t Context::moe_grouped_q80(int il, int T) {
    const HParams &hp = model->hp;
    const LayerWeights &L = model->layers[(size_t)il];
    const int E = hp.n_embd, FF = hp.n_ff, KU = hp.n_expert_used, NE = hp.n_expert, GR = T * KU;
    HIP_TRY(launch_moe_gather_act(aq_e_, moe_tok_, GR, E, aq_eg_, stream_));
    prep_owner_ = nullptr;
    const uint8_t *w_gu[2] = {L.gate_exps.planes, L.up_exps.planes}, *w_d[1] = {L.down_exps.planes};
    float *o_gu[2] = {ffn_g_, ffn_ug_}, *o_d[1] = {y_g_};
    HIP_TRY(launch_mmq_q80_moe(L.gate_exps.type, w_gu, o_gu, 2, L.gate_exps.planes_bytes / (size_t)L.gate_exps.n_expert, NE, moe_meta_, (int)L.gate_exps.N, E, GR, aq_eg_, FF, stream_));
    if (imx_on_) HIP_TRY(imx_collect(il, IMX_FFN_DOWN, ffn_g_, ffn_ug_, FF, GR, nullptr, moe_meta_));
    HIP_TRY(launch_swiglu_quant(ffn_g_, ffn_ug_, FF, GR, aq_ffg_, false, true, stream_, nullptr, nullptr));
    HIP_TRY(launch_mmq_q80_moe(L.down_exps.type, w_d, o_d, 1, L.down_exps.planes_bytes / (size_t)L.down_exps.n_expert, NE, moe_meta_, (int)L.down_exps.N, FF, GR, aq_ffg_, E, stream_));
    return launch_moe_scatter_combine(x_, y_g_, moe_w_, moe_slot_, T, E, KU, stream_);
}

hipError_t Context::moe_grouped_per_expert(int il, int T, bool q80_any) {
    const HParams &hp = model->hp;
    const LayerWeights &L = model->layers[(size_t)il];
    const int E = hp.n_embd, FF = hp.n_ff, KU = hp.n_expert_used, NE = hp.n_expert, GR = T * KU;
    HIP_TRY(hipMemcpyAsync(h_moe_meta_, moe_meta_, (size_t)(2 * NE + 1) * 4, hipMemcpyDeviceToHost, stream_));
    HIP_TRY(launch_moe_gather_act(aq_e_, moe_tok_, GR, E, aq_eg_, stream_));
    prep_owner_ = nullptr;
    HIP_TRY(hipStreamSynchronize(stream_));
    auto view = [](const DevTensor &w, int e) {
        DevTensor v = w;
        v.data = w.data + (size_t)e * w.row_bytes * (size_t)w.N;
        v.n_expert = 1;
        v.planes = w.planes ? w.planes + (size_t)e * (w.planes_bytes / (size_t)w.n_expert) : nullptr;
        return v;
    };
    auto rows = [](const ActQuant &q, int r0, int K) {
        ActQuant v;
        if (q.qs) { v.qs = q.qs + (size_t)r0 * K; v.d = q.d + (size_t)r0 * (K / 256); v.bsums = q.bsums + (size_t)r0 * (K / 16); }
        if (q.qs0) { v.qs0 = q.qs0 + (size_t)r0 * K; v.d0 = q.d0 + (size_t)r0 * (K / 32); }
        return v;
    };
    auto copy_batch = [&](const DevTensor &w, int e, const ActQuant &q, int K, int n_e, float *out, int ld_out) {
        return launch_mmq_q80(w.planes + (size_t)e * (w.planes_bytes / (size_t)w.n_expert), mmq_q80_copy_row_bytes(w.type, K), (int)w.N, K, n_e, q, out, ld_out, nullptr, stream_,
                              mmq_q80_copy_form(w.type), true);
    };
    const bool pl_gu = !act_is_q80(L.gate_exps.type) || !act_is_q80(L.up_exps.type), pl_d = !act_is_q80(L.down_exps.type);
    if (pl_gu) HIP_TRY(launch_mmq_prep(aq_eg_, E, GR, mmq_bh_, mmq_bl_, stream_));
    hipError_t e_exp = hipSuccess;
    for (int e = 0; e < NE && e_exp == hipSuccess; e++) {
        const int n_e = h_moe_meta_[e], r0 = h_moe_meta_[NE + e];
        if (n_e <= 0) continue;
        if (pl_gu) { bh_over_ = mmq_bh_ + (size_t)r0 * (E >> 4); bl_over_ = mmq_bl_ + (size_t)r0 * (E >> 4); }
        if (q80_any) {
            e_exp = copy_batch(L.gate_exps, e, rows(aq_eg_, r0, E), E, n_e, ffn_g_ + (size_t)r0 * FF, FF);
            if (e_exp == hipSuccess) e_exp = copy_batch(L.up_exps, e, rows(aq_eg_, r0, E), E, n_e, ffn_ug_ + (size_t)r0 * FF, FF);
            continue;
        }
        e_exp = linear(view(L.gate_exps, e), rows(aq_eg_, r0, E), nullptr, E, n_e, ffn_g_ + (size_t)r0 * FF, FF, nullptr, EPI_STORE);
        if (e_exp == hipSuccess) e_exp = linear(view(L.up_exps, e), rows(aq_eg_, r0, E), nullptr, E, n_e, ffn_ug_ + (size_t)r0 * FF, FF, nullptr, EPI_STORE);
    }
    bh_over_ = bl_over_ = nullptr;
    HIP_TRY(e_exp);
    if (imx_on_) HIP_TRY(imx_collect(il, IMX_FFN_DOWN, ffn_g_, ffn_ug_, FF, GR, nullptr, moe_meta_));
    HIP_TRY(launch_swiglu_quant(ffn_g_, ffn_ug_, FF, GR, aq_ffg_, !act_is_q80(L.down_exps.type), act_is_q80(L.down_exps.type), stream_,
                                pl_d ? mmq_bh_ : nullptr, pl_d ? mmq_bl_ : nullptr));
    prep_owner_ = nullptr;
    for (int e = 0; e < NE && e_exp == hipSuccess; e++) {
        const int n_e = h_moe_meta_[e], r0 = h_moe_meta_[NE + e];
        if (n_e <= 0) continue;
        if (pl_d) { bh_over_ = mmq_bh_ + (size_t)r0 * (FF >> 4); bl_over_ = mmq_bl_ + (size_t)r0 * (FF >> 4); }
        if (q80_any) { e_exp = copy_batch(L.down_exps, e, rows(aq_ffg_, r0, FF), FF, n_e, y_g_ + (size_t)r0 * E, E); continue; }
        e_exp = linear(view(L.down_exps, e), rows(aq_ffg_, r0, FF), nullptr, FF, n_e, y_g_ + (size_t)r0 * E, E, nullptr, EPI_STORE);
    }
    bh_over_ = bl_over_ = nullptr;
    HIP_TRY(e_exp);
    return launch_moe_scatter_combine(x_, y_g_, moe_w_, moe_slot_, T, E, KU, stream_);
}

hipError_t Context::moe_selected(int il, int T) {
    const HParams &hp = model->hp;
    const LayerWeights &L = model->layers[(size_t)il];
    const int E = hp.n_embd, FF = hp.n_ff, KU = hp.n_expert_used;
    MMVQArgs a{}, d{};
    if (T == 1 && moe_selected_desc(il, a, d)) {
        HIP_TRY(launch_mmvq(a, stream_));
        HIP_TRY(launch_mmvq(d, stream_));
        return launch_moe_combine(x_, moe_out_, moe_w_, T, E, KU, (size_t)T * E, stream_);
    }
    const bool fuse_q = type_is_kq456(L.down_exps.type) && (FF % 256) == 0 && mmvq_fast_kb_ok((FF + 2047) / 2048);
    for (int t = 0; t < T; t++) {
        for (int j = 0; j < KU; j++) {
            const int32_t *esel = moe_ids_ + (size_t)t * KU + j;
            a = MMVQArgs{};
            a.n_seg = 2; a.K = E; a.T = 1; a.epi = EPI_SWIGLU;
            a.seg[0] = make_seg(L.gate_exps, ffn_ + (size_t)t * FF, FF, nullptr, esel);
            a.seg[1] = make_seg(L.up_exps, ffn_u_ + (size_t)t * FF, FF, nullptr, esel);
            chunk_act(a, aq_e_, E, t);
            if (L.gate_exps.type == L.up_exps.type) {
                HIP_TRY(launch_mmvq(a, stream_));
            } else {
                a.epi = EPI_STORE;
                HIP_TRY(launch_mmvq(a, stream_));
                HIP_TRY(launch_swiglu(ffn_ + (size_t)t * FF, ffn_u_ + (size_t)t * FF, ffn_ + (size_t)t * FF, FF, stream_));
            }
            if (!fuse_q) { HIP_TRY(launch_quantize(ffn_ + (size_t)t * FF, FF, 1, aq_ff_, !act_is_q80(L.down_exps.type), act_is_q80(L.down_exps.type), stream_)); prep_owner_ = nullptr; }
            d = MMVQArgs{};
            d.n_seg = 1; d.K = FF; d.T = 1; d.epi = EPI_STORE;
            if (fuse_q) { d.fuse_mode = 2; d.nx = ffn_ + (size_t)t * FF; }
            d.seg[0] = make_seg(L.down_exps, moe_out_ + ((size_t)j * T + t) * E, E, nullptr, esel);
            chunk_act(d, aq_ff_, FF, 0);
            HIP_TRY(launch_mmvq(d, stream_));
        }
    }
    return launch_moe_combine(x_, moe_out_, moe_w_, T, E, KU, (size_t)T * E, stream_);
}

hipError_t Context::ffn_moe(int il, const Step &st) {
    const HParams &hp = model->hp;
    const LayerWeights &L = model->layers[(size_t)il];
    const int E = hp.n_embd, FF = hp.n_ff, T = st.T, KU = hp.n_expert_used;
    HIP_TRY(launch_rmsnorm_quant(x_, (const float *)L.ffn_norm.data, E, T, hp.eps, xn_, &aq_e_,
                                 !act_is_q80(L.gate_exps.type) || !act_is_q80(L.up_exps.type), act_is_q80(L.gate_exps.type) || act_is_q80(L.up_exps.type), stream_));
    prep_owner_ = nullptr;
    prof_mark("norm_quant");
    const int32_t *forced = moe_forced_T_ == T ? d_moe_forced_ + (size_t)il * T * KU : nullptr;
    if ((L.gate_inp.type == T_F32 || L.gate_inp.type == T_F16) && hp.n_expert <= 8) {
        HIP_TRY(launch_moe_router(L.gate_inp.type, L.gate_inp.data, hp.n_expert, E, xn_, T, KU, router_, moe_ids_, moe_w_, stream_, forced));
    } else {
        HIP_TRY(launch_mmv_float(L.gate_inp.type, L.gate_inp.data, hp.n_expert, E, xn_, T, router_, hp.n_expert, nullptr, stream_));
        HIP_TRY(launch_moe_route(router_, T, hp.n_expert, KU, moe_ids_, moe_w_, stream_, forced));
    }
    prof_mark("moe_route");
    const bool exps_q = type_is_quant(L.gate_exps.type) && type_is_quant(L.up_exps.type) && type_is_quant(L.down_exps.type);
    if (imx_on_) HIP_TRY(imx_collect(il, IMX_ROUTER, xn_, nullptr, E, T, nullptr, nullptr));
    if (exps_q && (T >= g_moe_group_min || imx_on_) && aq_eg_.qs) {
        HIP_TRY(launch_moe_group(moe_ids_, T, KU, hp.n_expert, moe_meta_, moe_slot_, moe_tok_, stream_));
        if (imx_on_) HIP_TRY(imx_collect(il, IMX_FFN_IN, xn_, nullptr, E, T * KU, moe_tok_, moe_meta_));
        const bool one_launch = T >= 32 && L.gate_exps.planes && L.up_exps.planes && L.down_exps.planes && L.gate_exps.type == L.up_exps.type &&
                                L.gate_exps.N == L.up_exps.N && mmq_planes_moe_ok(L.gate_exps.type, (int)L.gate_exps.N, E) &&
                                mmq_planes_moe_ok(L.down_exps.type, (int)L.down_exps.N, FF) && (L.gate_exps.N % 64) == 0;
        const bool q80_ok = T >= 32 && L.gate_exps.planes && L.up_exps.planes && L.down_exps.planes && L.gate_exps.type == T_MXFP4 && L.up_exps.type == T_MXFP4 &&
                            L.down_exps.type == T_MXFP4 && L.gate_exps.N == L.up_exps.N && mmq_q80_moe_ok(T_MXFP4, (int)L.gate_exps.N, E) &&
                            mmq_q80_moe_ok(T_MXFP4, (int)L.down_exps.N, FF) && aq_eg_.qs0 && aq_ffg_.qs0;
        if (q80_ok && g_moe_q80_grouped) HIP_TRY(moe_grouped_q80(il, T));
        else HIP_TRY(one_launch ? moe_grouped_one_launch(il, T) : moe_grouped_per_expert(il, T, q80_ok));
    } else {
        HIP_TRY(moe_selected(il, T));
    }
    prof_mark("moe_ffn");
    return hipSuccess;
}

hipError_t Context::ffn_block(int il, const Step &st) {
    if (model->hp.n_expert > 0) return ffn_moe(il, st);
    bool quantised = false;
    HIP_TRY(ffn_dense_gate_up(il, st, quantised));
    HIP_TRY(ffn_down(il, st, quantised));
    if (st.tp) HIP_TRY(tp_reduce_into_x(st.T));
    prof_mark("ffn_down");
    return hipSuccess;
}

hipError_t Context::tap_layer(int il, int T) {
    if (!debug_taps_ || !dbg_) return hipSuccess;
    return hipMemcpyAsync(dbg_ + (size_t)il * cp.n_ubatch * model->hp.n_embd, x_, (size_t)T * model->hp.n_embd * 4, hipMemcpyDeviceToDevice, stream_);
}

hipError_t Context::run_layers(int T, int n_kv_cap) {
    if (model->hp.encoder) return run_layers_encoder(T, n_kv_cap);
    cur_T_ = T;
    const HParams &hp = model->hp;
    const int E = hp.n_embd, FF = hp.n_ff;
    Step st = step_constants(T, n_kv_cap);
    att_splits_ = flash_attn_pick_splits(T, hp.n_head_kv, st.n_kv_max);

    bool mega = T == 1 && !profile_ && !debug_taps_ && !ub_embd_ && lora_.empty() && !imx_on_ && mega_prepare();
    AttnArgs ma{};
    if (mega) {
        ma = attn_args(0, 1, st.n_kv_max, d_pos_);
        ma.out_q = &aq_o_; ma.out_q8k = !act_is_q80(model->layers[0].wo.type); ma.out_q80 = false;
        ma.splits = flash_attn_decode_splits(st.n_kv_max);
        if (st.chunk_lists) attn_chunk_lists(ma);
        mega = flash_attn_decode_fused_applicable(ma, st.ra_step);
    }
    st.engine = T == 1 && !mega && !profile_ && !debug_taps_ && !ub_embd_ && lora_.empty() && !imx_on_ && engine_prepare();
    last_layers_engine_ = st.engine;
    HIP_TRY(launch_step_setup_embed(d_pos_, T, st.ra_step, rope_cs_, d_cell_pos_, d_cell_seq_, d_cell_, d_seqmask_, mega ? d_mega_sync_ : nullptr,
                                    d_step_serial_, model->tok_embd.type, model->tok_embd.data, E, d_tok_, x_, stream_));
    if (ub_embd_) HIP_TRY(hipMemcpyAsync(x_, ub_embd_, (size_t)T * E * sizeof(float), hipMemcpyHostToDevice, stream_));
    prof_mark("embed");
    last_layers_mega_ = mega;
    if (mega)
        return launch_decode_mega(d_mega_layers_, hp.n_layer, (E + 2047) >> 11, (FF + 2047) >> 11, ma, rope_cs_, st.ra_step.n_rot, k_, v_, d_cell_,
                                  att_counters_, d_mega_sync_, h_mega_flag_, d_mega_probe_, mega_lds_, stream_);

    for (int il = 0; il < hp.n_layer; il++) {
        const AttnPlan ap = plan_attn(il, st);
        HIP_TRY(attn_qkv(il, st, ap));
        HIP_TRY(attn_core(il, st, ap));
        if (st.engine) {
            HIP_TRY(launch_decode_engine(d_engine_layers_ + il, E, FF, d_engine_gran_, d_engine_epoch_, il, il == engine_probe_layer_ ? d_engine_probe_ : nullptr, stream_));
        } else {
            HIP_TRY(attn_output(il, st, ap));
            if (st.tp) HIP_TRY(tp_reduce_into_x(T));
            prof_mark("attn_out");
            HIP_TRY(ffn_block(il, st));
        }
        HIP_TRY(tap_layer(il, T));
    }
    return hipSuccess;
}

hipError_t Context::tp_reduce_into_x(int T) {
    return tp_all_reduce_sum(tp_part_, x_, (size_t)T * model->hp.n_embd, stream_);
}

hipError_t Context::run_output(int n_out, int out_base) {
    logits_on_host_ = false;
    if (n_out <= 0) return hipSuccess;
    const HParams &hp = model->hp;
    const int E = hp.n_embd, V = hp.n_vocab;
    float *const xo = cur_T_ == 1 && n_out == 1 ? x_ : xo_;
    if (xo != x_) HIP_TRY(launch_gather_rows_f32(x_, d_outrow_, n_out, E, xo_, stream_));
    if (hp.encoder) {
        HIP_TRY(hipMemcpyAsync(d_embd_ + (size_t)out_base * E, xo, (size_t)n_out * E * 4, hipMemcpyDeviceToDevice, stream_));
        prof_mark("embd");
        return hipSuccess;
    }
    if (embeddings_enabled) {
        HIP_TRY(launch_rmsnorm_quant(xo, (const float *)model->out_norm.data, E, n_out, hp.eps, d_embd_ + (size_t)out_base * E, nullptr, false, false, stream_));
        prof_mark("embd");
        return hipSuccess;
    }
    const bool oq = type_is_quant(model->output.type);
    const bool imx_head = imx_on_ && imx_output_;
    const bool lora_head = lora_on(-1, LORA_OUTPUT);
    const bool head_rows = lora_head || imx_head;
    static const bool zc_env = !(getenv("MI355_LOGITS_ZERO_COPY") && getenv("MI355_LOGITS_ZERO_COPY")[0] == '0');
    logits_on_host_ = zc_env && oq && cur_T_ == 1 && n_out == 1 && cp.logits_to_host && !hp.tp_exchange && h_logits_ != nullptr && !head_rows;
    if (oq && can_fuse(E, n_out) && !head_rows) {
        pending_fuse_.mode = 1; pending_fuse_.x = xo; pending_fuse_.w = (const float *)model->out_norm.data; pending_fuse_.eps = hp.eps;
    } else {
        prep_owner_ = nullptr;
        HIP_TRY(launch_rmsnorm_quant(xo, (const float *)model->out_norm.data, E, n_out, hp.eps, oq && !head_rows ? nullptr : xn_, &aq_e_,
                                     oq && !act_is_q80(model->output.type), act_is_q80(model->output.type), stream_));
        prof_mark("norm_quant");
        if (imx_head) HIP_TRY(imx_collect(-1, IMX_QKV, xn_, nullptr, E, n_out, nullptr, nullptr));
    }
    float *lg = d_logits_ + (size_t)out_base * V;
    const int VL = hp.n_vocab_local, P = hp.tp_size;
    if (hp.tp_exchange && VL * P == V) {
        if (n_out > 1 && (size_t)n_out > tp_logits_rows_) {
            HIP_TRY(hipStreamSynchronize(stream_));
            tp_logits_ = (float *)dalloc((size_t)n_out * V * 4);
            if (!tp_logits_) return hipErrorOutOfMemory;
            tp_logits_rows_ = (size_t)n_out;
            HIP_TRY(hipDeviceSynchronize());
        }
        float *gathered = n_out == 1 ? lg : tp_logits_;
        float *part = gathered + (size_t)hp.tp_rank * n_out * VL;
        HIP_TRY(linear(model->output, aq_e_, xn_, E, n_out, part, VL, nullptr, EPI_STORE));
        pending_fuse_ = Fuse();
        HIP_TRY(tp_all_gather(part, gathered, (size_t)n_out * VL, stream_));
        for (int r = 0; r < P && n_out > 1; r++)
            HIP_TRY(hipMemcpy2DAsync(lg + (size_t)r * VL, (size_t)V * 4, tp_logits_ + (size_t)r * n_out * VL, (size_t)VL * 4, (size_t)VL * 4, (size_t)n_out,
                                     hipMemcpyDeviceToDevice, stream_));
    } else {
        if (logits_on_host_) pending_fuse_.out_host = h_logits_ + (size_t)out_base * V;
        HIP_TRY(linear(model->output, aq_e_, xn_, E, n_out, lg, V, nullptr, EPI_STORE));
        if (lora_head) {
            const int target = LORA_OUTPUT;
            HIP_TRY(lora_add(-1, &target, &lg, &V, 1, xn_, E, E, n_out));
        }
    }
    pending_fuse_ = Fuse();
    prof_mark("lm_head");
    for (int r0 = 0; r0 < n_out; r0 += (int)cp.n_ubatch) {
        const int nr = std::min((int)cp.n_ubatch, n_out - r0);
        HIP_TRY(launch_argmax_rows(lg + (size_t)r0 * V, V, nr, h_argmax_ + out_base + r0, argmax_scratch_, (int)cp.n_ubatch, stream_));
    }
    prof_mark("argmax");
    return hipSuccess;
}

int Context::decode_ubatch(int n, const int32_t *tokens, const int32_t *pos, const int32_t *seq, const uint64_t *seqmask,
                           const int8_t *flags, int out_base) {
    { const unsigned long long ls = next_launch_serial(); if (!first_unchecked_launch_) first_unchecked_launch_ = ls; }
    cur_max_pos_ = 0;
    for (int i = 0; i < n; i++) cur_max_pos_ = std::max(cur_max_pos_, (int)pos[i]);
    std::vector<int> tcell;
    if (!alloc_cells(n, seqmask, tcell)) return 1;
    for (int i = 0; i < n; i++) {
        KVCell &c = cells_[(size_t)tcell[(size_t)i]];
        c.pos = pos[i]; c.seqs = seqmask[i]; c.delta = 0;
    }
    int hi = 0;
    for (int i = (int)cells_.size() - 1; i >= 0; i--) if (cells_[(size_t)i].pos >= 0) { hi = i + 1; break; }
    n_kv_ = std::min((int)cp.n_ctx, (hi + 31) & ~31);

    if (meta_dirty_) {
        std::vector<int32_t> cpos(cells_.size());
        std::vector<uint64_t> cseq(cells_.size());
        for (size_t i = 0; i < cells_.size(); i++) { cpos[i] = cells_[i].pos; cseq[i] = cells_[i].seqs; }
        if (hipMemcpyAsync(d_cell_pos_, cpos.data(), cpos.size() * 4, hipMemcpyHostToDevice, stream_) != hipSuccess ||
            hipMemcpyAsync(d_cell_seq_, cseq.data(), cseq.size() * 8, hipMemcpyHostToDevice, stream_) != hipSuccess ||
            hipStreamSynchronize(stream_) != hipSuccess) { last_error = "cell table upload failed"; return -1; }
        meta_dirty_ = false;
    }
    if (stage_event_) (void)hipEventSynchronize(stage_event_);
    const size_t T = ((size_t)cp.n_ubatch + 1) & ~(size_t)1;
    int32_t *h_nkv = (int32_t *)h_stage_;
    int32_t *h_tok = (int32_t *)(h_stage_ + 16), *h_pos = h_tok + T, *h_seq = h_pos + T, *h_cell = h_seq + T, *h_out = h_cell + T;
    uint64_t *h_mask = (uint64_t *)(h_out + T);
    h_nkv[0] = n_kv_;
    int n_out = 0;
    for (int i = 0; i < n; i++) {
        h_tok[i] = tokens[i]; h_pos[i] = pos[i]; h_seq[i] = seq[i]; h_cell[i] = tcell[(size_t)i]; h_mask[i] = seqmask[i];
        if (flags[i]) h_out[n_out++] = i;
    }
    if (hipMemcpyAsync(d_stage_, h_stage_, stage_bytes_, hipMemcpyHostToDevice, stream_) != hipSuccess) { last_error = "token upload failed"; return -1; }
    chunk_lmax_ = 0;
    batch_distinct_ = n >= 2 && n <= 64;
    {
        uint64_t seen = 0;
        for (int i = 0; i < n && batch_distinct_; i++) {
            const uint64_t mk = seqmask[i];
            if (mk == 0 || (mk & (mk - 1)) != 0 || (seen & mk) != 0) batch_distinct_ = false;
            seen |= mk;
        }
    }
    bool lists_usable = false;
    {
        const HParams &hp = model->hp;
        RopeArgs ra = rope_args(*model, false);
        AttnArgs aa{};
        aa.T = n; aa.H = hp.n_head; aa.G = hp.n_head_kv; aa.D = hp.head_dim; aa.n_kv_max = n_kv_; aa.type_k = cp.type_k; aa.type_v = cp.type_v;
        lists_usable = n <= 64 && flash_attn_decode_applicable(aa, ra) && kv_store_fast_applicable(aa.G, aa.D, cp.type_k, cp.type_v, ra);
    }
    if ((n >= 2 || cp.n_seq_max > 1) && lists_usable) {
        chunk_lmax_ = build_attn_chunk_lists(n_kv_, (int)cells_.size(), [&](int i, int32_t &p, uint64_t &m) { p = cells_[(size_t)i].pos; m = cells_[(size_t)i].seqs; },
                                             seq, n, chunk_stride_, h_chunks_, h_chunks_ + (size_t)64 * chunk_stride_);
        if (hipMemcpyAsync(d_chunks_, h_chunks_, (size_t)64 * (chunk_stride_ + 1) * 4, hipMemcpyHostToDevice, stream_) != hipSuccess) { last_error = "chunk list upload failed"; return -1; }
    }
    static const bool profiler_safe = getenv("MI355_PROFILER_SAFE") && getenv("MI355_PROFILER_SAFE")[0] == '1';
    if (profiler_safe) (void)hipStreamSynchronize(stream_);
    if (!stage_event_) (void)hipEventCreateWithFlags(&stage_event_, hipEventDisableTiming);
    if (stage_event_) (void)hipEventRecord(stage_event_, stream_);

    const int V = model->hp.n_vocab;
    if (n == 1 && !model->hp.encoder && !ub_embd_) { (void)mega_prepare(); (void)engine_prepare(); }
    attn_out_skip_step_ = n == 1 && !attn_out_off_ && !model->hp.encoder && !fused_acquire();
    if (attn_out_skip_step_) fused_skipped_steps++;
    bool graph_ok = cp.use_graphs && n == 1 && n_out == 1 && out_base == 0 && !profile_ && !debug_taps_ && !embeddings_enabled && moe_forced_T_ == 0 && !ub_embd_ && !attn_out_skip_step_ && !imx_on_;
    hipError_t e = hipSuccess;
    if (graph_ok) {
        int bucket = std::min((int)cp.n_ctx, (n_kv_ + 255) & ~255);
        chunk_cap_ = 0;
        if (chunk_lmax_ > 0) {
            chunk_cap_ = attn_chunk_grid(chunk_lmax_, chunk_stride_);
            bucket = -chunk_cap_;
        }
        auto git = graphs_.find(bucket);
        graph_exec_ = git == graphs_.end() ? nullptr : git->second;
        if (!graph_exec_) {
            hipGraph_t g = nullptr;
            std::string inner;
            e = hipStreamBeginCapture(stream_, hipStreamCaptureModeThreadLocal);
            if (e == hipSuccess) {
                last_error.clear();
                hipError_t e2 = run_layers(1, bucket > 0 ? bucket : std::min((int)cp.n_ctx, chunk_cap_ * 64));
                if (e2 == hipSuccess) e2 = run_output(1, 0);
                if (e2 == hipSuccess && cp.logits_to_host && !logits_on_host_) e2 = hipMemcpyAsync(h_logits_, d_logits_, (size_t)V * 4, hipMemcpyDeviceToHost, stream_);
                if (e2 != hipSuccess) inner = last_error;
                e = hipStreamEndCapture(stream_, &g);
                if (e2 != hipSuccess) e = e2;
            }
            if (e == hipSuccess) e = hipGraphInstantiate(&graph_exec_, g, nullptr, nullptr, 0);
            if (g) (void)hipGraphDestroy(g);
            if (e != hipSuccess && model->hp.tp_exchange) {
                (void)hipGetLastError();
                cp.use_graphs = false;
                graph_ok = false;
                graph_exec_ = nullptr;
                e = hipSuccess;
            } else {
                if (e != hipSuccess) { last_error = std::string("graph capture failed: ") + hipGetErrorString(e) + (inner.empty() ? "" : " / " + inner); return -1; }
                graphs_[bucket] = graph_exec_;
                graph_is_mega_[graph_exec_] = last_layers_mega_;
                graph_is_engine_[graph_exec_] = last_layers_engine_;
            }
        }
        if (graph_ok) e = hipGraphLaunch(graph_exec_, stream_);
    }
    if (!graph_ok) {
        prof_begin();
        chunk_cap_ = chunk_lmax_;
        e = run_layers(n, n_kv_);
        if (e == hipSuccess) e = run_output(n_out, out_base);
        if (profiler_safe) (void)hipStreamSynchronize(stream_);
        if (e == hipSuccess && n_out > 0 && cp.logits_to_host && !embeddings_enabled && !logits_on_host_)
            e = hipMemcpyAsync(h_logits_ + (size_t)out_base * V, d_logits_ + (size_t)out_base * V, (size_t)n_out * V * 4, hipMemcpyDeviceToHost, stream_);
        prof_end();
    }
    if (e != hipSuccess) { last_error = std::string("decode failed: ") + hipGetErrorString(e) + " / " + last_error_string(); return -1; }
    if (n == 1 && (graph_ok ? graph_is_mega_[graph_exec_] : last_layers_mega_)) mega_steps++;
    if (n == 1 && (graph_ok ? graph_is_engine_[graph_exec_] : last_layers_engine_)) engine_steps++;
    dbg_tokens_ = n;
    return 0;
}

namespace {
struct RoctxApi {
    int (*push)(const char *) = nullptr;
    int (*pop)() = nullptr;
    RoctxApi() {
        const char *ev = getenv("MI355_ROCTX");
        if (!ev || ev[0] != '1') return;
        for (const char *n : {"librocprofiler-sdk-roctx.so.1", "librocprofiler-sdk-roctx.so", "libroctx64.so.4", "libroctx64.so"}) {
            if (void *h = dlopen(n, RTLD_NOW | RTLD_GLOBAL)) {
                push = reinterpret_cast<int (*)(const char *)>(dlsym(h, "roctxRangePushA"));
                pop = reinterpret_cast<int (*)()>(dlsym(h, "roctxRangePop"));
                if (push && pop) return;
                push = nullptr; pop = nullptr;
            }
        }
    }
};
struct TraceRange {
    static RoctxApi &api() { static RoctxApi a; return a; }
    bool on = false;
    TraceRange(const char *what, int n) {
        if (!api().push) return;
        char buf[96];
        snprintf(buf, sizeof buf, "mi355_decode %s n=%d", what, n);
        api().push(buf);
        on = true;
    }
    ~TraceRange() { if (on) api().pop(); }
};
}

int Context::decode(int n_tokens, const int32_t *tokens, const int32_t *pos, const int32_t *n_seq_id, int32_t *const *seq_id,
                    const int8_t *logits_flags, const float *embd) {
    if (n_tokens <= 0) { last_error = "empty batch"; return -1; }
    const TraceRange trace_range(embd ? "embeddings" : n_tokens == 1 ? "step" : n_tokens <= 64 ? "steps" : "prompt", n_tokens);
    std::vector<int32_t> no_tokens;
    if (embd) {
        if (model->hp.encoder) { last_error = "an encoder model takes token ids, not embeddings"; return -1; }
        if (tokens) { last_error = "a batch carries token ids or embeddings, not both"; return -1; }
        if (!pos) { last_error = "an embeddings batch needs positions"; return -1; }
        no_tokens.assign((size_t)n_tokens, 0);
        tokens = no_tokens.data();
    } else if (!tokens) { last_error = "batch without tokens"; return -1; }
    if (hipSetDevice(model->device) != hipSuccess) return -1;
    const HParams &hp = model->hp;
    if (hp.encoder && (size_t)n_tokens > cp.n_ubatch) { last_error = "encoder model: a batch of " + std::to_string(n_tokens) + " tokens does not fit one micro-batch (n_ubatch " + std::to_string(cp.n_ubatch) + ")"; return -1; }
    if (has_shift_) apply_k_shift();
    if (debug_taps_ && !dbg_) dbg_ = (float *)dalloc((size_t)hp.n_layer * cp.n_ubatch * hp.n_embd * 4);

    std::vector<int32_t> seq((size_t)n_tokens);
    std::vector<uint64_t> mask((size_t)n_tokens);
    std::vector<int8_t> flags((size_t)n_tokens);
    int n_out = 0;
    out_row_of_batch_.assign((size_t)n_tokens, -1);
    for (int i = 0; i < n_tokens; i++) {
        if (tokens[i] < 0 || tokens[i] >= hp.n_vocab) { last_error = "token id " + std::to_string(tokens[i]) + " out of range [0, " + std::to_string(hp.n_vocab) + ")"; return -1; }
        if (pos && pos[i] < 0) { last_error = "negative position " + std::to_string(pos[i]) + " for token " + std::to_string(i); return -1; }
        uint64_t mk = 0;
        const int ns = n_seq_id ? n_seq_id[i] : 1;
        for (int j = 0; j < ns; j++) {
            const int s = seq_id ? seq_id[i][j] : 0;
            if (s < 0 || s >= 64) { last_error = "seq id " + std::to_string(s) + " out of range [0, 64)"; return -1; }
            mk |= 1ull << s;
        }
        seq[(size_t)i] = seq_id ? seq_id[i][0] : 0;
        mask[(size_t)i] = mk;
        flags[(size_t)i] = logits_flags ? (logits_flags[i] != 0) : (i == n_tokens - 1);
        if (flags[(size_t)i]) out_row_of_batch_[(size_t)i] = n_out++;
    }
    if ((size_t)n_out > logits_cap_rows_) {
// ... 356 lines not shown
        if (topk_scratch_) (void)hipFree(topk_scratch_);
        if (d_topk_adj_) (void)hipFree(d_topk_adj_);
        if (h_topk_) (void)hipHostFree(h_topk_);
        if (h_topk_adj_) (void)hipHostFree(h_topk_adj_);
        topk_scratch_ = nullptr; d_topk_adj_ = nullptr; h_topk_ = nullptr; h_topk_adj_ = nullptr; topk_rows_cap_ = 0;
        const int cap = std::max(n, std::min(64, (int)cp.n_seq_max));
        const size_t adj_bytes = (size_t)cap * sizeof(TopkAdj) + (size_t)cap * sizeof(int);
        if (hipMalloc(&topk_scratch_, topk_scratch_bytes(V) * (size_t)cap) != hipSuccess || hipMalloc((void **)&d_topk_adj_, adj_bytes) != hipSuccess ||
            hipHostMalloc((void **)&h_topk_, (size_t)cap * TOPK_MAX_K * sizeof(unsigned long long), hipHostMallocDefault) != hipSuccess ||
            hipHostMalloc((void **)&h_topk_adj_, adj_bytes, hipHostMallocDefault) != hipSuccess) { last_error = "top-k workspace allocation failed"; return -1; }
        topk_rows_cap_ = cap;
    }
    TopkAdj *ha = reinterpret_cast<TopkAdj *>(h_topk_adj_);
    int *hr = reinterpret_cast<int *>(h_topk_adj_ + (size_t)topk_rows_cap_ * sizeof(TopkAdj));
    for (int r = 0; r < n; r++) {
        TopkAdj &d = ha[r];
        const TopkAdj &a = adjs[r];
        d.n = a.n; d.repeat = a.repeat; d.freq = a.freq; d.present = a.present;
        memcpy(d.tok, a.tok, (size_t)a.n * sizeof(int)); memcpy(d.bias, a.bias, (size_t)a.n * sizeof(float)); memcpy(d.cnt, a.cnt, (size_t)a.n * sizeof(int));
        hr[r] = rows[(size_t)r];
    }
    const size_t rows_off = (size_t)topk_rows_cap_ * sizeof(TopkAdj);
    if (hipMemcpyAsync(d_topk_adj_, h_topk_adj_, (size_t)n * sizeof(TopkAdj), hipMemcpyHostToDevice, stream_) != hipSuccess ||
        hipMemcpyAsync(d_topk_adj_ + rows_off, h_topk_adj_ + rows_off, (size_t)n * sizeof(int), hipMemcpyHostToDevice, stream_) != hipSuccess) { last_error = "top-k staging failed"; return -1; }
    if (launch_topk_rows(d_logits_, V, n, reinterpret_cast<const int *>(d_topk_adj_ + rows_off), kmax, reinterpret_cast<const TopkAdj *>(d_topk_adj_), topk_scratch_, h_topk_,
                         stream_) != hipSuccess) { last_error = "top-k launch failed"; return -1; }
    if (hipStreamSynchronize(stream_) != hipSuccess || !mega_check() || !stream_check()) return -1;
    for (int r = 0; r < n; r++)
        for (int j = 0; j < ks[r]; j++) {
            const unsigned long long key = h_topk_[(size_t)r * TOPK_MAX_K + (size_t)j];
            unsigned u = (unsigned)(key >> 32);
            u ^= (u >> 31) ? 0x80000000u : 0xffffffffu;
            float f;
            memcpy(&f, &u, 4);
            toks[(size_t)r * TOPK_MAX_K + (size_t)j] = (int32_t)(0xffffffffu - (unsigned)(key & 0xffffffffull));
            logits[(size_t)r * TOPK_MAX_K + (size_t)j] = f;
        }
    return n;
}

int Context::topk_ith(int i, int k, const TopkAdj &adj, int32_t *toks, float *logits) {
    int32_t t[TOPK_MAX_K];
    float l[TOPK_MAX_K];
    if (topk_rows(1, &i, &k, &adj, t, l) != 1) return -1;
    memcpy(toks, t, (size_t)k * sizeof(int32_t));
    memcpy(logits, l, (size_t)k * sizeof(float));
    return k;
}

int Context::debug_layer_out(int il, float *dst, size_t cap) {
    const HParams &hp = model->hp;
    if (!dbg_ || il < 0 || il >= hp.n_layer) return -1;
    const size_t n = (size_t)dbg_tokens_ * hp.n_embd;
    if (cap < n) return -1;
    (void)hipStreamSynchronize(stream_);
    if (hipMemcpy(dst, dbg_ + (size_t)il * cp.n_ubatch * hp.n_embd, n * 4, hipMemcpyDeviceToHost) != hipSuccess) return -1;
    return dbg_tokens_;
}

double Context::bench_weight_sweep(int iters, uint64_t *bytes_out, int *launches_out) {
    const HParams &hp = model->hp;
    const int E = hp.n_embd;
    if (hp.encoder) return -1.0;
    (void)hipMemsetAsync(x_, 0, (size_t)E * 4, stream_);
    uint64_t bytes = 0; int launches = 0;
    Step st = step_constants(1, 64);
    st.chunk_lists = false;
    st.out = xo_;
    struct ProfileOff { bool &p; bool was; ~ProfileOff() { p = was; } } profile_off{profile_, profile_};
    profile_ = false;
    auto sweep = [&](bool count) -> hipError_t {
        for (int il = 0; il < hp.n_layer; il++) {
            const LayerWeights &L = model->layers[(size_t)il];
            const AttnPlan ap = plan_attn(il, st);
            HIP_TRY(attn_qkv(il, st, ap));
            HIP_TRY(attn_output(il, st, ap));
            if (count) {
                bytes += (ap.qkv_in_attn ? 0 : L.wq.ggml_bytes + L.wk.ggml_bytes + L.wv.ggml_bytes) + (ap.ao_form ? 0 : L.wo.ggml_bytes);
                launches += (ap.qkv_in_attn ? 0 : 1) + (ap.ao_form ? 0 : 1);
            }
            if (hp.n_expert > 0) {
                const int KU = hp.n_expert_used;
                MMVQArgs a{}, d{};
                if (!moe_ids_ || !moe_selected_desc(il, a, d)) continue;
                if (count) { std::vector<int32_t> ids((size_t)KU); for (int j = 0; j < KU; j++) ids[(size_t)j] = j; HIP_TRY(hipMemcpy(moe_ids_, ids.data(), ids.size() * 4, hipMemcpyHostToDevice)); }
                HIP_TRY(launch_mmvq(a, stream_));
                HIP_TRY(launch_mmvq(d, stream_));
                if (count) {
                    bytes += (L.gate_exps.ggml_bytes + L.up_exps.ggml_bytes + L.down_exps.ggml_bytes) / (uint64_t)L.gate_exps.n_expert * (uint64_t)KU;
                    launches += 2;
                }
                continue;
            }
            bool quantised = false;
            int n_down = 0;
            HIP_TRY(ffn_dense_gate_up(il, st, quantised));
            HIP_TRY(ffn_down(il, st, quantised, &n_down));
            if (count) {
                bytes += L.gate.ggml_bytes + L.up.ggml_bytes + L.down.ggml_bytes;
                launches += 1 + n_down;
            }
        }
        if (type_is_quant(model->output.type) && can_fuse(E, 1)) { pending_fuse_.mode = 1; pending_fuse_.x = x_; pending_fuse_.w = (const float *)model->out_norm.data; pending_fuse_.eps = hp.eps; }
        HIP_TRY(linear(model->output, aq_e_, xn_, E, 1, d_logits_, (int)model->output.N, nullptr, EPI_STORE));
        pending_fuse_ = Fuse();
        if (count) { bytes += model->output.ggml_bytes; launches += 1; }
        return hipSuccess;
    };
    if (!d_logits_) { d_logits_ = (float *)dalloc((size_t)hp.n_vocab * 4); logits_cap_rows_ = 0; }
    if (sweep(true) != hipSuccess) return -1.0;
    hipEvent_t e0, e1;
    (void)hipEventCreate(&e0); (void)hipEventCreate(&e1);
    (void)hipStreamSynchronize(stream_);
    hipGraph_t g = nullptr; hipGraphExec_t ge = nullptr;
    bool graphed = cp.use_graphs && hipStreamBeginCapture(stream_, hipStreamCaptureModeThreadLocal) == hipSuccess;
    if (graphed) {
        const hipError_t es = sweep(false);
        const hipError_t ec = hipStreamEndCapture(stream_, &g);
        graphed = es == hipSuccess && ec == hipSuccess && g && hipGraphInstantiate(&ge, g, nullptr, nullptr, 0) == hipSuccess;
        if (graphed) { (void)hipGraphLaunch(ge, stream_); (void)hipStreamSynchronize(stream_); }
    }
    (void)hipEventRecord(e0, stream_);
    for (int i = 0; i < iters; i++) {
        if (graphed) { if (hipGraphLaunch(ge, stream_) != hipSuccess) return -1.0; }
        else if (sweep(false) != hipSuccess) return -1.0;
    }
    (void)hipEventRecord(e1, stream_);
    (void)hipEventSynchronize(e1);
    float ms = 0;
    (void)hipEventElapsedTime(&ms, e0, e1);
    (void)hipEventDestroy(e0); (void)hipEventDestroy(e1);
    if (ge) (void)hipGraphExecDestroy(ge);
    if (g) (void)hipGraphDestroy(g);
    if (bytes_out) *bytes_out = bytes;
    if (launches_out) *launches_out = launches;
    return (double)ms * 1000.0 / iters;
}

}
```

cortex.llamacpp_amd/host/runtime.h:

```cpp
#pragma once

#include <hip/hip_runtime.h>

#include <cstdint>
#include <map>
#include <memory>
#include <string>
#include <vector>

#include "../csrc/kernels.h"
#include "gguf.h"
#include "lora.h"
#include "model_plan.h"

namespace mi355 {

struct LoraAdapter;
struct Model : ModelLayout {
    std::unique_ptr<GGUFFile> file;
    std::vector<LoraAdapter *> adapters;
    std::string path, desc;
    int device = 0;
    std::vector<uint8_t *> arenas;
    uint64_t device_bytes = 0, host_bytes = 0, file_tensor_bytes = 0, bytes_per_token = 0, planes_bytes = 0;
    ~Model();
};

Model *model_load(const std::string &path, int main_gpu, std::string &err, int &status, int prefill_planes = -1, int tp_rank = 0, int tp_size = 1);

struct LoraPair { int layer, target, type, r; int64_t K, N; const uint8_t *A, *B; };
struct LoraAdapter {
    Model *model = nullptr;
    std::string path;
    float alpha = 0.0f;
    std::vector<LoraPair> pairs;
    std::vector<int> index;
    uint8_t *arena = nullptr;
    uint64_t device_bytes = 0;
    const LoraPair *find(int layer, int target) const {
        const size_t i = (size_t)(layer + 1) * LORA_N_TARGETS + (size_t)target;
        return i < index.size() && index[i] >= 0 ? &pairs[(size_t)index[i]] : nullptr;
    }
};
LoraAdapter *lora_load(Model *m, const std::string &path, std::string &err, int &status);
void lora_free(LoraAdapter *a);

struct KVCell {
    int32_t pos = -1;
    int32_t delta = 0;
    uint64_t seqs = 0;
};

void debug_raise_stream_error(unsigned code);
struct ContextParams {
    uint32_t n_ctx = 512, n_batch = 2048, n_ubatch = 512, n_seq_max = 1;
    int type_k = T_F16, type_v = T_F16;
    bool flash_attn = true, embeddings = false, use_graphs = true;
    bool logits_to_host = true;
};

struct ProfileEntry { std::string name; float us; };

struct Fuse {
    int mode = 0;
    const float *x = nullptr, *w = nullptr;
    float eps = 0.0f;
    float *out_host = nullptr;
};

struct MMVQTrace {
    struct Rec { int T, kernel; MMVQStreamForm form; };
    std::vector<Rec> recs;
    void note(const MMVQArgs &a);
};
MMVQSeg make_seg(const DevTensor &w, float *out, int ld_out, const float *resid, const int32_t *esel);
MMVQArgs single_token_desc(int n_seg, int K, int epi, int fuse, const float *nx, const float *nw, float eps, const ActQuant &aq);
hipError_t mmvq_tokens(MMVQSeg *segs, int n_seg, int K, int T, int epi, const ActQuant &aq, hipStream_t st, const Fuse &fz = Fuse(), MMVQTrace *trace = nullptr);
enum { PM_NONE = 0, PM_KSPLIT = 1, PM_PLANES = 2, PM_FLY = 3 };
enum { PM_ROLE_ONE = 0, PM_ROLE_MULTI = 1, PM_ROLE_GATE_UP = 2 };
struct PromptMatmul {
    int form = PM_NONE;
    int n_fused = 0;
    bool swiglu = false;
    bool planes_only = false;
    bool need_prep = false;
};
PromptMatmul prompt_mul_mat_choice(int role, const DevTensor *const *ws, int n, int K, int T, MMQWorkspace wsp);
unsigned *install_stream_error_word();

void set_moe_q80_grouped(bool on);
void set_moe_group_min(int tokens);
void set_attn_store_fuse(bool on);
void set_rope_fast(bool on);
void set_decode_engine(int on);
void set_decode_mega(bool on);

class Context {
  public:
    int64_t engine_steps = 0;
    int64_t qkv_attn_launches = 0;
    int64_t fused_skipped_steps = 0;
    int64_t mega_steps = 0;
    Context(Model *m, const ContextParams &p);
    ~Context();
    bool init(std::string &err);

    int decode(int n_tokens, const int32_t *tokens, const int32_t *pos, const int32_t *n_seq_id, int32_t *const *seq_id,
               const int8_t *logits_flags, const float *embd = nullptr);
    float *logits_ith(int i);
    float *embeddings_ith(int i);
    int32_t argmax_ith(int i);
    int32_t argmax_prob_ith(int i, float *p);
    int spec_verify(int n_groups, const int32_t *group_start, const int32_t *draft, int32_t *ids_out, int32_t *n_accept_out);
    int token_logprobs(int n, const int32_t *batch_rows, const int32_t *targets, float *logprob_out, int32_t *rank_out);
    int logits_kl(Context &base, int n, const int32_t *rows_base, const int32_t *rows_self, float *kl_out, int32_t *same_top_out);
    struct PplStats {
        int64_t n_chunks = 0, count = 0, top1 = 0, dead = 0, same_top = 0;
        int32_t has_base = 0, stopped = 0;
        double nll = 0, nll2 = 0, nll_base = 0, nll2_base = 0, kl = 0, kl2 = 0;
    };
    int perplexity(const int32_t *tokens, int64_t n_tokens, int n_chunk, int32_t bos, int seq, Context *base, float *logprob_out, float *kl_out,
                   int (*cb)(const PplStats &, void *), void *user, PplStats &out);
    int imatrix_begin(bool process_output);
    int imatrix_end();
    int imatrix_clear();
    bool imatrix_on() const { return imx_on_; }
    int imatrix_n_entries() const { return (int)imx_names_.size(); }
    bool imatrix_entry(int i, std::string &name, int &ne0, int &n_mat) const;
    int imatrix_get(int i, float *sum2, int32_t *counts);
    int force_moe_ids(const int32_t *ids, int n_layer, int T, int k);
    int topk_ith(int i, int k, const TopkAdj &adj, int32_t *toks, float *logits);
    int topk_rows(int n, const int *is, const int *ks, const TopkAdj *adjs, int32_t *toks, float *logits);
    void synchronize();

    int set_adapter_lora(LoraAdapter *a, float scale);
    int rm_adapter_lora(LoraAdapter *a);
    void clear_adapter_lora();

    void kv_clear();
    bool kv_seq_rm(int seq, int p0, int p1);
    void kv_seq_cp(int src, int dst, int p0, int p1);
    void kv_seq_add(int seq, int p0, int p1, int delta);
    int kv_used_cells() const;

    static constexpr uint32_t STATE_MAGIC = 0x564b354du, STATE_VERSION = 1, STATE_HEADER_BYTES = 32;
    size_t state_seq_size(int seq) const;
    size_t state_seq_get(int seq, uint8_t *dst, size_t cap);
    size_t state_seq_set(int seq, const uint8_t *src, size_t len);
    float state_ms_pack = 0, state_ms_copy = 0, state_ms_unpack = 0;
    bool state_timing = false;

    int debug_layer_out(int il, float *dst, size_t cap);
    void set_debug_taps(bool on) { debug_taps_ = on; }
    void set_profile(bool on) { profile_ = on; }
    const std::vector<ProfileEntry> &last_profile() const { return last_profile_; }
    double bench_weight_sweep(int iters, uint64_t *bytes, int *launches = nullptr);

    Model *model;
    ContextParams cp;
    uint64_t device_bytes = 0;
    std::string last_error;
    bool embeddings_enabled = false;

  private:
    struct Bufs;
    const float *ub_embd_ = nullptr;
    int decode_ubatch(int n, const int32_t *tokens, const int32_t *pos, const int32_t *seq, const uint64_t *seqmask,
                      const int8_t *flags, int out_base);
    int find_slot(int n);
    bool alloc_cells(int n, const uint64_t *seqmask, std::vector<int> &out);
    std::vector<int> region_next_;
    void apply_k_shift();
    uint8_t *d_state_stage_ = nullptr;
    size_t state_stage_bytes_ = 0;
    int32_t *d_state_cells_ = nullptr;
    KVLayerView *d_state_layers_ = nullptr;
    bool state_prepare();
    const char *state_refusal() const;
    size_t state_cell_bytes() const;
    struct Step {
        int T = 0, n_kv_max = 0;
        RopeArgs ra_step{};
        bool engine = false;
        bool tp = false;
        bool chunk_lists = false;
        int attn_mode = 2;
        bool rope_fast = true, fuse_down_env = true;
        float *out = nullptr;
        const float *resid = nullptr;
    };
    struct AttnPlan {
        RopeArgs ra;
        AttnArgs aa, af;
        MMVQSeg ao_seg;
        int ao_epi;
        QKVFuse qf;
        bool qkv_float, qkv_prologue;
        bool o_planes;
        bool decode_attn, fused_step;
        bool ao_form, qkv_in_attn;
        bool qkv_lora;
    };
    Step step_constants(int T, int n_kv_cap) const;
    AttnArgs attn_args(int il, int T, int n_kv_max, const int32_t *tok_pos) const;
    void attn_chunk_lists(AttnArgs &aa) const;
    AttnPlan plan_attn(int il, const Step &st) const;
    hipError_t attn_qkv(int il, const Step &st, const AttnPlan &p);
    hipError_t attn_core(int il, const Step &st, const AttnPlan &p);
    hipError_t attn_output(int il, const Step &st, const AttnPlan &p);
    hipError_t ffn_block(int il, const Step &st);
    hipError_t ffn_moe(int il, const Step &st);
    bool moe_selected_desc(int il, MMVQArgs &a, MMVQArgs &d) const;
    hipError_t moe_grouped_one_launch(int il, int T);
    hipError_t moe_grouped_per_expert(int il, int T, bool q80_any = false);
    hipError_t moe_grouped_q80(int il, int T);
    hipError_t moe_selected(int il, int T);
    hipError_t ffn_dense_gate_up(int il, const Step &st, bool &quantised);
    hipError_t quantise_for_down(int il, int T, bool combined, bool planes_any_T);
    hipError_t ffn_down(int il, const Step &st, bool quantised, int *n_matvec = nullptr);
    hipError_t tap_layer(int il, int T);
    hipError_t run_layers(int T, int n_kv_cap);
    hipError_t run_layers_encoder(int T, int n_kv_cap);
    hipError_t run_output(int n_out, int out_base);
    hipError_t linear(const DevTensor &w, const ActQuant &aq, const float *x_f32, int K, int T, float *out, int ld_out,
                      const float *resid, int epi);
    hipError_t linear_multi(const DevTensor *const *ws, float *const *outs, int n, const ActQuant &aq, const float *x_f32, int T, const float *const *bias = nullptr,
                            bool *bias_done = nullptr);
    hipError_t linear_bf16(const DevTensor *const *ws, float *const *outs, const float *const *bias, int n, int K, int T, int ld_out, const float *resid, int epi);
    struct ActiveLora { LoraAdapter *a; float scale; };
    std::vector<ActiveLora> lora_;
    float *lora_t_ = nullptr;
    bool lora_on(int layer, int target) const;
    bool lora_changed();
    hipError_t lora_add(int layer, const int *targets, float *const *outs, const int *lds, int n, const float *x, int ld_x, int K, int T);
    enum { IMX_QKV = 0, IMX_O = 1, IMX_FFN_IN = 2, IMX_FFN_DOWN = 3, IMX_ROUTER = 4, IMX_SLOTS = 5 };
    struct ImxAcc { int K = 0, n_mat = 0; float *sum2 = nullptr; int32_t *count = nullptr; };
    struct ImxName { std::string name; int acc; };
    std::vector<ImxAcc> imx_acc_;
    std::vector<ImxName> imx_names_;
    bool imx_on_ = false, imx_output_ = false;
    uint8_t *imx_block_ = nullptr;
    size_t imx_block_bytes_ = 0, imx_acc_bytes_ = 0;
    float *imx_slabs_ = nullptr;
    size_t imx_slab_floats_ = 0;
    bool f32_rows(int layer, int target) const { return imx_on_ || lora_on(layer, target); }
    hipError_t imx_collect(int il, int slot, const float *x, const float *x2, int K, int R, const int32_t *row_src, const int32_t *meta);
    void prof_mark(const char *name);
    void prof_begin();
    void prof_end();
    void *dalloc(size_t bytes);

    hipStream_t stream_ = nullptr;
    int cur_T_ = 0;
    std::vector<void *> allocs_;
    std::vector<KVCell> cells_;
    int head_ = 0;
    bool has_shift_ = false;
    bool meta_dirty_ = true;

    std::vector<KVLayerView> kv_;
    int32_t *d_cell_pos_ = nullptr;
    uint64_t *d_cell_seq_ = nullptr;
    int32_t *d_delta_ = nullptr;
    int32_t *d_pos_open_ = nullptr;
    int32_t *d_tok_ = nullptr, *d_pos_ = nullptr, *d_seq_ = nullptr, *d_cell_ = nullptr, *d_nkv_ = nullptr, *d_outrow_ = nullptr;
    uint64_t *d_seqmask_ = nullptr;
    uint8_t *h_stage_ = nullptr;
    size_t stage_bytes_ = 0;
    uint8_t *d_stage_ = nullptr;
    hipEvent_t stage_event_ = nullptr;
    float *x_ = nullptr, *xn_ = nullptr, *q_ = nullptr, *k_ = nullptr, *v_ = nullptr, *att_ = nullptr, *ffn_ = nullptr, *ffn_u_ = nullptr;
    float *xo_ = nullptr, *router_ = nullptr, *moe_out_ = nullptr;
    uint16_t *xb_ = nullptr;
    float *tp_part_ = nullptr, *tp_logits_ = nullptr;
    size_t tp_logits_rows_ = 0;
    hipError_t tp_reduce_into_x(int T);
    int32_t *moe_ids_ = nullptr;
    float *moe_w_ = nullptr;
    ActQuant aq_eg_, aq_ffg_;
    float *ffn_g_ = nullptr, *ffn_ug_ = nullptr, *y_g_ = nullptr;
    int32_t *moe_meta_ = nullptr, *moe_slot_ = nullptr, *moe_tok_ = nullptr, *h_moe_meta_ = nullptr;
    ActQuant aq_e_, aq_ff_, aq_o_;
    int8_t *mmq_bh_ = nullptr, *mmq_bl_ = nullptr;
    MMQWorkspace mmq_ws_;
    const void *prep_owner_ = nullptr;
    int prep_K_ = 0, prep_T_ = 0;
    hipError_t ensure_prep(const ActQuant &aq, int K, int T);
    void prep_written(const ActQuant &aq, int K, int T) { prep_owner_ = aq.qs; prep_K_ = K; prep_T_ = T; }
    bool batch_distinct_ = false;
    const int8_t *bh_over_ = nullptr, *bl_over_ = nullptr;
    float *att_part_ = nullptr;
    size_t att_part_floats_ = 0;
    int cur_max_pos_ = 0;
    float *d_embd_ = nullptr, *h_embd_ = nullptr;
    bool embd_fetched_ = false, last_was_embd_ = false;
    int32_t *h_chunks_ = nullptr, *d_chunks_ = nullptr;
    int chunk_stride_ = 0, chunk_lmax_ = 0, chunk_cap_ = 0;
    MegaLayer *d_mega_layers_ = nullptr;
    unsigned *d_mega_sync_ = nullptr;
    int *h_mega_flag_ = nullptr;
    unsigned long long *d_mega_probe_ = nullptr;
    size_t mega_lds_ = 0;
    bool last_layers_mega_ = false;
    std::map<hipGraphExec_t, bool> graph_is_mega_, graph_is_engine_;
    bool last_layers_engine_ = false;
    int mega_state_ = 0;
    bool mega_prepare();
    bool mega_check();
    EngineLayer *d_engine_layers_ = nullptr;
    unsigned long long *d_engine_gran_ = nullptr;
    unsigned *d_engine_epoch_ = nullptr;
    unsigned long long *d_engine_probe_ = nullptr;
    int engine_probe_layer_ = -1;
    unsigned err_epoch_seen_ = 0;
    unsigned long long first_unchecked_launch_ = 0;
    bool logits_on_host_ = false;
    bool attn_out_off_ = false;
    int engine_state_ = 0;
    bool engine_prepare();
    bool fused_acquire();
    void fused_release();
    bool holds_fused_ = false, attn_out_skip_step_ = false;
    bool stream_check();
    int32_t *d_moe_forced_ = nullptr;
    int moe_forced_T_ = 0, moe_forced_cap_ = 0;
    unsigned *att_counters_ = nullptr;
    unsigned *d_step_serial_ = nullptr;
    unsigned long long *d_qkv_gran_ = nullptr;
    unsigned long long *d_ao_gran_ = nullptr;
    unsigned *d_ao_flags_ = nullptr;
    float *argmax_scratch_ = nullptr, *rope_cs_ = nullptr;
    void *topk_scratch_ = nullptr;
    uint8_t *d_topk_adj_ = nullptr, *h_topk_adj_ = nullptr;
    int topk_rows_cap_ = 0;
    float *spec_scratch_ = nullptr;
    int32_t *d_spec_in_ = nullptr, *h_spec_ = nullptr;
// ... 30 lines not shown
```

include/mi355_llama.h:

```cpp
#ifndef MI355_LLAMA_H
#define MI355_LLAMA_H

#include <stddef.h>
#include <stdint.h>

#ifdef __cplusplus
extern "C" {
#endif

#define MI355_API __attribute__((visibility("default")))

typedef struct mi355_model   mi355_model;
typedef struct mi355_context mi355_context;

typedef int32_t mi355_token;
typedef int32_t mi355_pos;
typedef int32_t mi355_seq_id;

enum mi355_status {
    MI355_OK            = 0,
    MI355_ERR_NO_DEVICE = -100,
    MI355_ERR_IO        = -101,
    MI355_ERR_FORMAT    = -102,
    MI355_ERR_ARG       = -103,
// ... 31 lines not shown
MI355_API int32_t  mi355_model_n_embd(const mi355_model *m);
MI355_API int32_t  mi355_model_n_layer(const mi355_model *m);
MI355_API int32_t  mi355_model_n_head(const mi355_model *m);
MI355_API int32_t  mi355_model_n_head_kv(const mi355_model *m);
MI355_API int32_t  mi355_model_n_ctx_train(const mi355_model *m);
MI355_API uint64_t mi355_model_size(const mi355_model *m);
MI355_API uint64_t mi355_model_cpu_buffer(const mi355_model *m);
MI355_API uint64_t mi355_model_other_buffer(const mi355_model *m);
MI355_API uint64_t mi355_model_bytes_per_token(const mi355_model *m);
MI355_API uint64_t mi355_model_planes_bytes(const mi355_model *m);
MI355_API const char *mi355_model_desc(const mi355_model *m);
MI355_API int mi355_model_meta_str(const mi355_model *m, const char *key, char *buf, size_t buf_size);

typedef struct mi355_context_params {
    uint32_t n_ctx;
    uint32_t n_batch;
    uint32_t n_ubatch;
    uint32_t n_seq_max;
    int32_t  type_k;
    int32_t  type_v;
    int32_t  flash_attn;
    int32_t  embeddings;
    int32_t  use_graphs;
    int32_t  logits_to_host;
} mi355_context_params;

MI355_API mi355_context_params mi355_context_default_params(void);
MI355_API mi355_context *mi355_context_new(mi355_model *model, mi355_context_params params);
MI355_API void           mi355_context_free(mi355_context *ctx);

MI355_API uint32_t mi355_n_ctx(const mi355_context *ctx);
MI355_API uint32_t mi355_n_batch(const mi355_context *ctx);
MI355_API uint32_t mi355_n_ubatch(const mi355_context *ctx);
MI355_API uint64_t mi355_context_device_bytes(const mi355_context *ctx);

typedef struct mi355_batch {
    int32_t        n_tokens;
    mi355_token   *token;
    float         *embd;
    mi355_pos     *pos;
    int32_t       *n_seq_id;
    mi355_seq_id **seq_id;
    int8_t        *logits;
} mi355_batch;

MI355_API mi355_batch mi355_batch_init(int32_t n_tokens, int32_t embd, int32_t n_seq_max);
MI355_API void        mi355_batch_free(mi355_batch batch);

MI355_API int32_t mi355_decode(mi355_context *ctx, mi355_batch batch);
MI355_API int32_t mi355_greedy_steps(mi355_context *ctx, mi355_token first, mi355_pos pos0, mi355_seq_id seq, int32_t n, mi355_token *out_tokens);
MI355_API float  *mi355_get_logits_ith(mi355_context *ctx, int32_t i);
MI355_API int32_t mi355_get_argmax_ith(mi355_context *ctx, int32_t i);
MI355_API int32_t mi355_get_argmax_prob_ith(mi355_context *ctx, int32_t i, float *p);
MI355_API int32_t mi355_spec_verify(mi355_context *ctx, int32_t n_groups, const int32_t *group_start, const mi355_token *draft, mi355_token *ids_out,
                                    int32_t *n_accept_out);
MI355_API int32_t mi355_speculative_steps(mi355_context *ctx_tgt, mi355_context *ctx_dft, mi355_token first, mi355_pos pos0, mi355_seq_id seq, int32_t n,
                                          int32_t n_max, int32_t n_min, float p_min, mi355_token *out_tokens, int64_t *stats);
MI355_API int32_t mi355_get_token_logprobs(mi355_context *ctx, int32_t n, const int32_t *batch_rows, const mi355_token *targets, float *logprob_out,
                                           int32_t *rank_out);
MI355_API int32_t mi355_logits_kl(mi355_context *ctx, mi355_context *ctx_base, int32_t n, const int32_t *rows_base, const int32_t *rows, float *kl_out,
                                  int32_t *same_top_out);
typedef struct mi355_ppl_stats {
    int64_t n_chunks, count, top1, dead, same_top;
    int32_t has_base, stopped;
    double  nll, nll2;
    double  nll_base, nll2_base, kl, kl2;
} mi355_ppl_stats;
typedef int32_t (*mi355_ppl_callback)(const mi355_ppl_stats *running, void *user);
MI355_API int32_t mi355_perplexity(mi355_context *ctx, mi355_context *ctx_base, const mi355_token *tokens, int64_t n_tokens, int32_t n_chunk, mi355_token bos,
                                   mi355_seq_id seq, float *logprob_out, float *kl_out, mi355_ppl_callback cb, void *user, mi355_ppl_stats *stats);
MI355_API int32_t mi355_imatrix_begin(mi355_context *ctx, int32_t process_output);
MI355_API int32_t mi355_imatrix_end(mi355_context *ctx);
MI355_API int32_t mi355_imatrix_clear(mi355_context *ctx);
MI355_API int32_t mi355_imatrix_n_entries(const mi355_context *ctx);
MI355_API int32_t mi355_imatrix_entry(const mi355_context *ctx, int32_t i, char *name_buf, int32_t cap, int32_t *ne0, int32_t *n_mat);
MI355_API int32_t mi355_imatrix_get(mi355_context *ctx, int32_t i, float *sum2, int32_t *counts);
MI355_API int32_t mi355_get_topk_ith(mi355_context *ctx, int32_t i, int32_t k, int32_t n_adj, const int32_t *adj_tok, const float *adj_bias,
                                     const int32_t *adj_count, float penalty_repeat, float penalty_freq, float penalty_present,
                                     int32_t *toks_out, float *logits_out);
MI355_API int64_t mi355_debug_mega_steps(const mi355_context *ctx);
MI355_API int64_t mi355_debug_engine_steps(const mi355_context *ctx);
MI355_API int64_t mi355_debug_fused_skipped_steps(const mi355_context *ctx);
MI355_API int64_t mi355_debug_qkv_attn_launches(const mi355_context *ctx);
MI355_API int64_t mi355_debug_qkv_attn_plan(int32_t type_q, int32_t type_k, int32_t type_v, int32_t type_o, int32_t n_embd, int32_t n_head, int32_t n_head_kv, int32_t head_dim,
                                            int32_t type_kv, int32_t n_kv, int32_t *slots_out);
MI355_API void    mi355_set_embeddings(mi355_context *ctx, int32_t enabled);
MI355_API float  *mi355_get_embeddings_ith(mi355_context *ctx, int32_t i);
MI355_API void    mi355_synchronize(mi355_context *ctx);

typedef struct mi355_adapter_lora mi355_adapter_lora;
MI355_API mi355_adapter_lora *mi355_adapter_lora_init(mi355_model *model, const char *path);
MI355_API void    mi355_adapter_lora_free(mi355_adapter_lora *adapter);
MI355_API float   mi355_adapter_lora_alpha(const mi355_adapter_lora *adapter);
MI355_API int32_t mi355_adapter_lora_n_pairs(const mi355_adapter_lora *adapter);
MI355_API int32_t mi355_set_adapter_lora(mi355_context *ctx, mi355_adapter_lora *adapter, float scale);
MI355_API int32_t mi355_rm_adapter_lora(mi355_context *ctx, mi355_adapter_lora *adapter);
MI355_API void    mi355_clear_adapter_lora(mi355_context *ctx);

MI355_API void    mi355_kv_cache_clear(mi355_context *ctx);
MI355_API int32_t mi355_kv_cache_seq_rm(mi355_context *ctx, mi355_seq_id seq, mi355_pos p0, mi355_pos p1);
MI355_API void    mi355_kv_cache_seq_cp(mi355_context *ctx, mi355_seq_id src, mi355_seq_id dst, mi355_pos p0, mi355_pos p1);
MI355_API void    mi355_kv_cache_seq_add(mi355_context *ctx, mi355_seq_id seq, mi355_pos p0, mi355_pos p1, mi355_pos delta);
MI355_API int32_t mi355_kv_cache_used_cells(const mi355_context *ctx);

MI355_API size_t mi355_state_seq_get_size(mi355_context *ctx, mi355_seq_id seq);
MI355_API size_t mi355_state_seq_get_data(mi355_context *ctx, uint8_t *dst, size_t cap, mi355_seq_id seq);
MI355_API size_t mi355_state_seq_set_data(mi355_context *ctx, const uint8_t *src, size_t len, mi355_seq_id dst);
MI355_API size_t mi355_state_seq_save_file(mi355_context *ctx, const char *path, mi355_seq_id seq, const mi355_token *tokens, size_t n_tokens);
MI355_API size_t mi355_state_seq_load_file(mi355_context *ctx, const char *path, mi355_seq_id dst_seq, mi355_token *tokens_out, size_t cap, size_t *n_tokens_out);
MI355_API void    mi355_debug_state_seq_timing(mi355_context *ctx, float out_ms[3]);

MI355_API void    mi355_debug_enable_taps(mi355_context *ctx, int32_t enabled);
MI355_API int32_t mi355_debug_layer_out(mi355_context *ctx, int32_t il, float *dst, size_t dst_floats);


MI355_API int mi355_op_quantize_act(int32_t act_type, const float *x, int64_t n_per_row, int64_t n_rows, void *out_blocks);
MI355_API int mi355_op_rms_norm_quant(const float *x, const float *w, int64_t n, int64_t T, float eps, float *y_f32, void *out_blocks);
MI355_API int mi355_op_swiglu_quant(const float *gate, const float *up, int64_t n, int64_t T, void *out_blocks);
MI355_API int mi355_op_mul_mat(int32_t type, const void *W, int64_t N, int64_t K, const float *x, int64_t T,
                               float *y, int32_t *isum, int32_t *msum);
MI355_API int mi355_op_mul_mat_add(int32_t type, const void *W, int64_t N, int64_t K, const float *x, int64_t T, const float *resid, float *y);
MI355_API int mi355_op_mul_mat_fused(int32_t type, const void *W, int64_t N, int64_t K, const float *x, const float *norm_w, float eps, float *y);
MI355_API int mi355_op_mat_vec_step(int32_t n_seg, const int32_t *types, const void *const *W, const int64_t *N, int64_t K, const float *x, int64_t T, int32_t epi,
                                    const float *resid, int32_t fuse, const float *norm_w, float eps, int32_t want_host_copy, int32_t n_sel, int32_t n_expert,
                                    const int32_t *expert_ids, int64_t ld_pad, float *const *y, float *y_host, int32_t *path);
MI355_API int mi355_op_prompt_mul_mat(int32_t n_seg, const int32_t *types, const void *const *W, const int64_t *N, int64_t K, const float *x, int64_t T, int32_t epi,
                                      const float *resid, int32_t in_place, int32_t prologue, const float *norm_w, float eps, int32_t form, int64_t ld_pad,
                                      float *const *y, int32_t *path);
MI355_API int mi355_op_act_q8k_planes(int32_t producer, const float *x, const float *x2, const float *norm_w, float eps, int64_t n, int64_t T, void *out_blocks,
                                      int8_t *out_bh, int8_t *out_bl, int8_t *prep_bh, int8_t *prep_bl, float *y_f32);
MI355_API int mi355_op_f32_to_bf16(const float *x, int64_t n, uint16_t *out);
MI355_API int mi355_op_mul_mat_bf16(int32_t n_seg, const void *const *W, const int64_t *N, int64_t K, const float *x, int64_t T, const float *const *bias,
                                    const float *resid, int32_t epi, int32_t path, int32_t tokens_per_launch, int32_t use_graph, float *const *y);
MI355_API int mi355_op_ffn_gate_up(int32_t type, const void *Wg, const void *Wu, int64_t N, int64_t K, const float *x, int64_t T, float *y);
MI355_API int mi355_op_lora_delta(int32_t n_seg, const int32_t *type, const void *const *A, const void *const *B, const int32_t *r, const int64_t *N, const float *scale,
                                  const float *x, int64_t K, int64_t T, const int64_t *ld_out, float *const *out);
MI355_API int mi355_op_rms_norm_mul(const float *x, const float *w, int64_t n, int64_t T, float eps, float *y);
MI355_API int mi355_op_rope(float *x, int32_t n_head, int32_t head_dim, int32_t n_rot, const int32_t *pos, int64_t T,
                            float freq_base, float freq_scale, const float *freq_factors, int32_t neox);
MI355_API int mi355_op_rope_yarn(float *x, int32_t n_head, int32_t head_dim, int32_t n_rot, const int32_t *pos, int64_t T,
                                 float freq_base, float freq_scale, const float *freq_factors, int32_t neox,
                                 float ext_factor, float attn_factor, float corr_lo, float corr_hi);
MI355_API int mi355_op_get_rows(int32_t type, const void *table, int64_t row_elems, int64_t n_rows_table,
                                const int32_t *ids, int64_t n_ids, float *dst);
MI355_API int mi355_op_repack_rows(int32_t type, const void *src_rows, int64_t row_elems, int64_t n_rows, void *dst);
MI355_API int mi355_op_swiglu(const float *gate, const float *up, int64_t n, float *y);
MI355_API int mi355_op_soft_max(const float *x, const float *mask, int64_t n, int64_t rows, float scale, float *y);
MI355_API int mi355_op_moe_route(const float *logits, int64_t T, int32_t n_expert, int32_t k, int32_t *ids, float *w);
MI355_API int mi355_op_moe_router(int32_t type, const void *gate_inp, int32_t n_expert, int64_t K, const float *x, int64_t T, int32_t k, int32_t fused,
                                  const int32_t *forced, float *logits, int32_t *ids, float *w);
MI355_API int mi355_op_argmax_rows(const float *x, int64_t n, const int32_t *launches, int32_t n_launch, int32_t cap_rows, int32_t *out);
MI355_API int mi355_op_argmax_prob_rows(const float *x, int64_t n, int32_t rows, int32_t *idx_out, float *p_out);
MI355_API int mi355_op_token_logprob_rows(const float *base, int64_t n, int32_t n_base_rows, const int32_t *rows, const int32_t *targets, int32_t R,
                                          float *logprob_out, int32_t *rank_out);
MI355_API int mi355_op_logits_kl_rows(const float *p, int32_t n_p_rows, const float *q, int32_t n_q_rows, int64_t n, const int32_t *rows_p, const int32_t *rows_q,
                                      int32_t R, float *kl_out, int32_t *same_top_out);
MI355_API int mi355_op_imatrix_accum(const float *x, const float *x2, int64_t ld, int64_t K, int32_t R, const int32_t *row_src, int32_t n_src_rows,
                                     const int32_t *counts_per_mat, int32_t n_mat, float *sum2_io, int32_t *count_io);
MI355_API int mi355_quantize_chunk(int32_t dst_type, int32_t src_type, const void *src, int64_t n_per_row, int64_t n_rows, const float *imatrix, void *dst);
MI355_API int mi355_quantize_supported(int32_t dst_type);
MI355_API int mi355_quantize_last_times(float *upload_ms, float *kernel_ms, float *download_ms);
MI355_API int mi355_op_spec_verify(const float *logits, int64_t n, int32_t n_base_rows, const int32_t *rows, int32_t R, const int32_t *group_start, int32_t G,
                                   const int32_t *draft, int32_t *ids_out, int32_t *n_accept_out);
MI355_API int mi355_op_topk_rows(const float *base, int64_t n, int32_t n_base_rows, const int32_t *rows, int32_t n_rows, int32_t k, const int32_t *adj_n,
                                 const int32_t *adj_tok, const float *adj_bias, const int32_t *adj_cnt, const float *repeat, const float *freq,
                                 const float *present, uint64_t *keys_out);
// ... 128 lines not shown
```

Before: 677.5.

## Compute last layer's attention output and FFN only for output rows

When a multi-token batch needs logits for only some rows, the last layer now gathers just those rows of the attention output and residual. It then runs the output projection and FFN on that subset, into the output buffer. This avoids last-layer O-proj and FFN work on rows whose hidden state is never read, mainly during prefill. Decode with T=1 is not affected, and the step struct now carries x/att pointers so the FFN and MoE paths can work on the reduced buffers.

```diff
diff --git a/cortex.llamacpp_amd/binding.py b/cortex.llamacpp_amd/binding.py
--- a/cortex.llamacpp_amd/binding.py
+++ b/cortex.llamacpp_amd/binding.py
@@ -101,6 +101,7 @@
     "mi355_debug_engine_steps": (C.c_int64, [_vp]),
     "mi355_debug_fused_skipped_steps": (C.c_int64, [_vp]),
     "mi355_debug_qkv_attn_launches": (C.c_int64, [_vp]),
+    "mi355_debug_last_layer_rows": (_i32, [_vp]),
     "mi355_debug_qkv_attn_plan": (C.c_int64, [C.c_int32] * 10 + [C.POINTER(C.c_int32)]),
     "mi355_set_embeddings": (None, [_vp, _i32]),
     "mi355_get_embeddings_ith": (C.POINTER(C.c_float), [_vp, _i32]),
@@ -1288,6 +1289,9 @@
     def qkv_attn_launches(self) -> int:
         return int(self.lib.mi355_debug_qkv_attn_launches(self.h))
 
+    def last_layer_rows(self) -> int:
+        return int(self.lib.mi355_debug_last_layer_rows(self.h))
+
     def engine_steps(self) -> int:
         return int(self.lib.mi355_debug_engine_steps(self.h))
 
diff --git a/cortex.llamacpp_amd/csrc/c_api.cc b/cortex.llamacpp_amd/csrc/c_api.cc
--- a/cortex.llamacpp_amd/csrc/c_api.cc
+++ b/cortex.llamacpp_amd/csrc/c_api.cc
@@ -438,6 +438,7 @@
 int64_t mi355_debug_engine_steps(const mi355_context *ctx) { return ctx->c->engine_steps; }
 int64_t mi355_debug_fused_skipped_steps(const mi355_context *ctx) { return ctx->c->fused_skipped_steps; }
 int64_t mi355_debug_qkv_attn_launches(const mi355_context *ctx) { return ctx->c->qkv_attn_launches; }
+int32_t mi355_debug_last_layer_rows(const mi355_context *ctx) { return ctx ? ctx->c->last_layer_rows() : -1; }
 int64_t mi355_debug_qkv_attn_plan(int32_t type_q, int32_t type_k, int32_t type_v, int32_t type_o, int32_t n_embd, int32_t n_head, int32_t n_head_kv, int32_t head_dim,
                                   int32_t type_kv, int32_t n_kv, int32_t *slots_out) {
     int slots = 0;
@@ -2424,6 +2425,7 @@
     if (!strcmp(name, "mmvq_stream")) { mmvq_set_stream(value != 0); return MI355_OK; }
     if (!strcmp(name, "attn_out_fused")) { set_attn_out_fused(value); return MI355_OK; }
     if (!strcmp(name, "qkv_attn_fused")) { set_qkv_attn_fused(value); return MI355_OK; }
+    if (!strcmp(name, "last_layer_rows")) { set_last_layer_rows(value); return MI355_OK; }
     if (!strcmp(name, "moe_group_min")) { set_moe_group_min(value); return MI355_OK; }
     if (!strcmp(name, "moe_q80_grouped")) { set_moe_q80_grouped(value != 0); return MI355_OK; }
     if (!strcmp(name, "fa_v_acc_f16")) { set_fa_v_acc_f16(value); return MI355_OK; }
diff --git a/cortex.llamacpp_amd/host/runtime.cc b/cortex.llamacpp_amd/host/runtime.cc
--- a/cortex.llamacpp_amd/host/runtime.cc
+++ b/cortex.llamacpp_amd/host/runtime.cc
@@ -1222,6 +1222,12 @@
 static bool g_rope_fast = true;
 void set_rope_fast(bool on) { g_rope_fast = on; }
 void set_decode_mega(bool on) { g_decode_mega = on ? 1 : 0; }
+static int g_last_layer_rows = -1;
+void set_last_layer_rows(int on) { g_last_layer_rows = on < 0 ? -1 : on ? 1 : 0; }
+static bool last_layer_rows_enabled() {
+    static const bool env_off = getenv("MI355_LAST_LAYER_ROWS") && getenv("MI355_LAST_LAYER_ROWS")[0] == '0';
+    return g_last_layer_rows < 0 ? !env_off : g_last_layer_rows > 0;
+}
 
 bool Context::mega_prepare() {
     if (mega_state_ != 0) return mega_state_ > 0;
@@ -1479,8 +1485,9 @@
     st.tp = hp.tp_exchange;
     st.chunk_lists = chunk_lmax_ > 0;
     st.attn_mode = attn_mode; st.rope_fast = rope_fast_env && g_rope_fast; st.fuse_down_env = fuse_down_env;
-    st.out = st.tp ? tp_part_ : x_;
-    st.resid = !st.tp || hp.tp_rank == 0 ? x_ : nullptr;
+    st.x = x_; st.att = att_;
+    st.out = st.tp ? tp_part_ : st.x;
+    st.resid = !st.tp || hp.tp_rank == 0 ? st.x : nullptr;
     return st;
 }
 
@@ -1509,7 +1516,7 @@
     p.qkv_prologue = !p.qkv_float && can_fuse(E, T) && !p.qkv_lora;
     AttnArgs &aa = p.aa;
     aa = attn_args(il, T, st.n_kv_max, d_pos_);
-    const bool o_q = type_is_quant(L.wo.type);
+    const bool o_q = type_is_quant(L.wo.type) && !(st.n_tail >= 0 && il == hp.n_layer - 1);
     aa.out_q = o_q ? &aq_o_ : nullptr; aa.out_q8k = !act_is_q80(L.wo.type); aa.out_q80 = act_is_q80(L.wo.type);
     p.o_planes = o_q && aa.out_q8k && T >= 3;
     if (p.o_planes) { aa.out_bh = mmq_bh_; aa.out_bl = mmq_bl_; }
@@ -1616,12 +1623,12 @@
 hipError_t Context::attn_output(int il, const Step &st, const AttnPlan &p) {
     const LayerWeights &L = model->layers[(size_t)il];
     if (p.ao_form) return hipSuccess;
-    HIP_TRY(linear(L.wo, aq_o_, att_, (int)L.wo.K, st.T, st.out, model->hp.n_embd, st.resid, p.ao_epi));
-    if (imx_on_) HIP_TRY(imx_collect(il, IMX_O, att_, nullptr, (int)L.wo.K, st.T, nullptr, nullptr));
+    HIP_TRY(linear(L.wo, aq_o_, st.att, (int)L.wo.K, st.T, st.out, model->hp.n_embd, st.resid, p.ao_epi));
+    if (imx_on_) HIP_TRY(imx_collect(il, IMX_O, st.att, nullptr, (int)L.wo.K, st.T, nullptr, nullptr));
     if (lora_on(il, LORA_O)) {
         const int target = LORA_O, ld = model->hp.n_embd;
         float *out = st.out;
-        HIP_TRY(lora_add(il, &target, &out, &ld, 1, att_, (int)L.wo.K, (int)L.wo.K, st.T));
+        HIP_TRY(lora_add(il, &target, &out, &ld, 1, st.att, (int)L.wo.K, (int)L.wo.K, st.T));
     }
     return hipSuccess;
 }
@@ -1649,10 +1656,10 @@
     const bool fuse_ffn = gq && uq && L.gate.type == L.up.type && can_fuse(E, T) && !lora_any;
     Fuse fz;
     if (fuse_ffn) {
-        fz.mode = 1; fz.x = x_; fz.w = (const float *)L.ffn_norm.data; fz.eps = hp.eps;
+        fz.mode = 1; fz.x = st.x; fz.w = (const float *)L.ffn_norm.data; fz.eps = hp.eps;
     } else {
         const bool pl = fk && T >= 3;
-        HIP_TRY(launch_rmsnorm_quant(x_, (const float *)L.ffn_norm.data, E, T, hp.eps, (!gq || !uq || lora_gu) ? xn_ : nullptr, &aq_e_, fk, f0, stream_,
+        HIP_TRY(launch_rmsnorm_quant(st.x, (const float *)L.ffn_norm.data, E, T, hp.eps, (!gq || !uq || lora_gu) ? xn_ : nullptr, &aq_e_, fk, f0, stream_,
                                      pl ? mmq_bh_ : nullptr, pl ? mmq_bl_ : nullptr));
         prep_owner_ = nullptr;
         if (pl) prep_written(aq_e_, E, T);
@@ -1749,13 +1756,13 @@
     return hipSuccess;
 }
 
-bool Context::moe_selected_desc(int il, MMVQArgs &a, MMVQArgs &d) const {
+bool Context::moe_selected_desc(int il, const float *x, MMVQArgs &a, MMVQArgs &d) const {
     const HParams &hp = model->hp;
     const LayerWeights &L = model->layers[(size_t)il];
     const int E = hp.n_embd, FF = hp.n_ff, KU = hp.n_expert_used;
     if (KU < 2 || KU > 8 || (int)cp.n_ubatch < KU || L.gate_exps.type != L.up_exps.type) return false;
     const bool prologue = can_fuse(E, 1) && !act_is_q80(L.gate_exps.type);
-    a = single_token_desc(2, E, EPI_SWIGLU, prologue ? 1 : 0, prologue ? x_ : nullptr, prologue ? (const float *)L.ffn_norm.data : nullptr, prologue ? hp.eps : 0.0f, aq_e_);
+    a = single_token_desc(2, E, EPI_SWIGLU, prologue ? 1 : 0, prologue ? x : nullptr, prologue ? (const float *)L.ffn_norm.data : nullptr, prologue ? hp.eps : 0.0f, aq_e_);
     a.n_sel = KU; a.sel_out_stride = FF;
     a.seg[0] = make_seg(L.gate_exps, ffn_, FF, nullptr, moe_ids_);
     a.seg[1] = make_seg(L.up_exps, ffn_u_, FF, nullptr, moe_ids_);
@@ -1765,10 +1772,10 @@
     return mmvq_fast_applicable(a) && mmvq_fast_applicable(d);
 }
 
-hipError_t Context::moe_grouped_one_launch(int il, int T) {
+hipError_t Context::moe_grouped_one_launch(int il, const Step &st) {
     const HParams &hp = model->hp;
     const LayerWeights &L = model->layers[(size_t)il];
-    const int E = hp.n_embd, FF = hp.n_ff, KU = hp.n_expert_used, NE = hp.n_expert, GR = T * KU;
+    const int E = hp.n_embd, FF = hp.n_ff, KU = hp.n_expert_used, NE = hp.n_expert, T = st.T, GR = T * KU;
     HIP_TRY(launch_moe_gather_act(aq_e_, moe_tok_, GR, E, aq_eg_, stream_));
     prep_owner_ = nullptr;
     const size_t ps_gu = L.gate_exps.planes_bytes / (size_t)L.gate_exps.n_expert, ps_d = L.down_exps.planes_bytes / (size_t)L.down_exps.n_expert;
@@ -1776,13 +1783,13 @@
     if (imx_on_) HIP_TRY(imx_collect(il, IMX_FFN_DOWN, ffn_g_, nullptr, FF, GR, nullptr, moe_meta_));
     HIP_TRY(launch_quantize(ffn_g_, FF, GR, aq_ffg_, true, false, stream_));
     HIP_TRY(launch_mmq_planes_moe(L.down_exps.type, L.down_exps.planes, ps_d, NE, moe_meta_, (int)L.down_exps.N, FF, GR, aq_ffg_, y_g_, E, stream_));
-    return launch_moe_scatter_combine(x_, y_g_, moe_w_, moe_slot_, T, E, KU, stream_);
-}
-
-hipError_t Context::moe_grouped_q80(int il, int T) {
+    return launch_moe_scatter_combine(st.x, y_g_, moe_w_, moe_slot_, T, E, KU, stream_);
+}
+
+hipError_t Context::moe_grouped_q80(int il, const Step &st) {
     const HParams &hp = model->hp;
     const LayerWeights &L = model->layers[(size_t)il];
-    const int E = hp.n_embd, FF = hp.n_ff, KU = hp.n_expert_used, NE = hp.n_expert, GR = T * KU;
+    const int E = hp.n_embd, FF = hp.n_ff, KU = hp.n_expert_used, NE = hp.n_expert, T = st.T, GR = T * KU;
     HIP_TRY(launch_moe_gather_act(aq_e_, moe_tok_, GR, E, aq_eg_, stream_));
     prep_owner_ = nullptr;
     const uint8_t *w_gu[2] = {L.gate_exps.planes, L.up_exps.planes}, *w_d[1] = {L.down_exps.planes};
@@ -1791,13 +1798,13 @@
     if (imx_on_) HIP_TRY(imx_collect(il, IMX_FFN_DOWN, ffn_g_, ffn_ug_, FF, GR, nullptr, moe_meta_));
     HIP_TRY(launch_swiglu_quant(ffn_g_, ffn_ug_, FF, GR, aq_ffg_, false, true, stream_, nullptr, nullptr));
     HIP_TRY(launch_mmq_q80_moe(L.down_exps.type, w_d, o_d, 1, L.down_exps.planes_bytes / (size_t)L.down_exps.n_expert, NE, moe_meta_, (int)L.down_exps.N, FF, GR, aq_ffg_, E, stream_));
-    return launch_moe_scatter_combine(x_, y_g_, moe_w_, moe_slot_, T, E, KU, stream_);
-}
-
-hipError_t Context::moe_grouped_per_expert(int il, int T, bool q80_any) {
+    return launch_moe_scatter_combine(st.x, y_g_, moe_w_, moe_slot_, T, E, KU, stream_);
+}
+
+hipError_t Context::moe_grouped_per_expert(int il, const Step &st, bool q80_any) {
     const HParams &hp = model->hp;
     const LayerWeights &L = model->layers[(size_t)il];
-    const int E = hp.n_embd, FF = hp.n_ff, KU = hp.n_expert_used, NE = hp.n_expert, GR = T * KU;
+    const int E = hp.n_embd, FF = hp.n_ff, KU = hp.n_expert_used, NE = hp.n_expert, T = st.T, GR = T * KU;
     HIP_TRY(hipMemcpyAsync(h_moe_meta_, moe_meta_, (size_t)(2 * NE + 1) * 4, hipMemcpyDeviceToHost, stream_));
     HIP_TRY(launch_moe_gather_act(aq_e_, moe_tok_, GR, E, aq_eg_, stream_));
     prep_owner_ = nullptr;
@@ -1849,18 +1856,18 @@
     }
     bh_over_ = bl_over_ = nullptr;
     HIP_TRY(e_exp);
-    return launch_moe_scatter_combine(x_, y_g_, moe_w_, moe_slot_, T, E, KU, stream_);
-}
-
-hipError_t Context::moe_selected(int il, int T) {
+    return launch_moe_scatter_combine(st.x, y_g_, moe_w_, moe_slot_, T, E, KU, stream_);
+}
+
+hipError_t Context::moe_selected(int il, const Step &st) {
     const HParams &hp = model->hp;
     const LayerWeights &L = model->layers[(size_t)il];
-    const int E = hp.n_embd, FF = hp.n_ff, KU = hp.n_expert_used;
+    const int E = hp.n_embd, FF = hp.n_ff, KU = hp.n_expert_used, T = st.T;
     MMVQArgs a{}, d{};
-    if (T == 1 && moe_selected_desc(il, a, d)) {
+    if (T == 1 && moe_selected_desc(il, st.x, a, d)) {
         HIP_TRY(launch_mmvq(a, stream_));
         HIP_TRY(launch_mmvq(d, stream_));
-        return launch_moe_combine(x_, moe_out_, moe_w_, T, E, KU, (size_t)T * E, stream_);
+        return launch_moe_combine(st.x, moe_out_, moe_w_, T, E, KU, (size_t)T * E, stream_);
     }
     const bool fuse_q = type_is_kq456(L.down_exps.type) && (FF % 256) == 0 && mmvq_fast_kb_ok((FF + 2047) / 2048);
     for (int t = 0; t < T; t++) {
@@ -1887,14 +1894,14 @@
             HIP_TRY(launch_mmvq(d, stream_));
         }
     }
-    return launch_moe_combine(x_, moe_out_, moe_w_, T, E, KU, (size_t)T * E, stream_);
+    return launch_moe_combine(st.x, moe_out_, moe_w_, T, E, KU, (size_t)T * E, stream_);
 }
 
 hipError_t Context::ffn_moe(int il, const Step &st) {
     const HParams &hp = model->hp;
     const LayerWeights &L = model->layers[(size_t)il];
     const int E = hp.n_embd, FF = hp.n_ff, T = st.T, KU = hp.n_expert_used;
-    HIP_TRY(launch_rmsnorm_quant(x_, (const float *)L.ffn_norm.data, E, T, hp.eps, xn_, &aq_e_,
+    HIP_TRY(launch_rmsnorm_quant(st.x, (const float *)L.ffn_norm.data, E, T, hp.eps, xn_, &aq_e_,
                                  !act_is_q80(L.gate_exps.type) || !act_is_q80(L.up_exps.type), act_is_q80(L.gate_exps.type) || act_is_q80(L.up_exps.type), stream_));
     prep_owner_ = nullptr;
     prof_mark("norm_quant");
@@ -1917,10 +1924,10 @@
         const bool q80_ok = T >= 32 && L.gate_exps.planes && L.up_exps.planes && L.down_exps.planes && L.gate_exps.type == T_MXFP4 && L.up_exps.type == T_MXFP4 &&
                             L.down_exps.type == T_MXFP4 && L.gate_exps.N == L.up_exps.N && mmq_q80_moe_ok(T_MXFP4, (int)L.gate_exps.N, E) &&
                             mmq_q80_moe_ok(T_MXFP4, (int)L.down_exps.N, FF) && aq_eg_.qs0 && aq_ffg_.qs0;
-        if (q80_ok && g_moe_q80_grouped) HIP_TRY(moe_grouped_q80(il, T));
-        else HIP_TRY(one_launch ? moe_grouped_one_launch(il, T) : moe_grouped_per_expert(il, T, q80_ok));
+        if (q80_ok && g_moe_q80_grouped) HIP_TRY(moe_grouped_q80(il, st));
+        else HIP_TRY(one_launch ? moe_grouped_one_launch(il, st) : moe_grouped_per_expert(il, st, q80_ok));
     } else {
-        HIP_TRY(moe_selected(il, T));
+        HIP_TRY(moe_selected(il, st));
     }
     prof_mark("moe_ffn");
     return hipSuccess;
@@ -1941,12 +1948,36 @@
     return hipMemcpyAsync(dbg_ + (size_t)il * cp.n_ubatch * model->hp.n_embd, x_, (size_t)T * model->hp.n_embd * 4, hipMemcpyDeviceToDevice, stream_);
 }
 
-hipError_t Context::run_layers(int T, int n_kv_cap) {
+hipError_t Context::last_layer_tail(int il, const Step &st) {
+    const HParams &hp = model->hp;
+    const LayerWeights &L = model->layers[(size_t)il];
+    const int n = st.n_tail, K = (int)L.wo.K;
+    if (n == 0) return hipSuccess;
+    HIP_TRY(launch_gather_rows_f32(att_, d_outrow_, n, K, q_, stream_));
+    HIP_TRY(launch_gather_rows_f32(x_, d_outrow_, n, hp.n_embd, xo_, stream_));
+    Step tl = step_constants(n, st.n_kv_max);
+    tl.x = tl.out = xo_; tl.resid = xo_; tl.att = q_;
+    if (type_is_quant(L.wo.type)) {
+        const bool k = !act_is_q80(L.wo.type), pl = k && n >= 3;
+        HIP_TRY(launch_quantize(tl.att, K, n, aq_o_, k, !k, stream_, pl ? mmq_bh_ : nullptr, pl ? mmq_bl_ : nullptr));
+        prep_owner_ = nullptr;
+        if (pl) prep_written(aq_o_, K, n);
+    }
+    AttnPlan ap{};
+    ap.ao_epi = EPI_ADD;
+    HIP_TRY(attn_output(il, tl, ap));
+    prof_mark("attn_out");
+    return ffn_block(il, tl);
+}
+
+hipError_t Context::run_layers(int T, int n_kv_cap, int n_out) {
+    tail_rows_ = -1;
     if (model->hp.encoder) return run_layers_encoder(T, n_kv_cap);
     cur_T_ = T;
     const HParams &hp = model->hp;
     const int E = hp.n_embd, FF = hp.n_ff;
     Step st = step_constants(T, n_kv_cap);
+    if (last_layer_rows_enabled() && T > 1 && n_out < T && !debug_taps_ && !imx_on_ && moe_forced_T_ == 0 && !st.tp) st.n_tail = n_out;
     att_splits_ = flash_attn_pick_splits(T, hp.n_head_kv, st.n_kv_max);
 
     bool mega = T == 1 && !profile_ && !debug_taps_ && !ub_embd_ && lora_.empty() && !imx_on_ && mega_prepare();
@@ -1973,7 +2004,10 @@
         const AttnPlan ap = plan_attn(il, st);
         HIP_TRY(attn_qkv(il, st, ap));
         HIP_TRY(attn_core(il, st, ap));
-        if (st.engine) {
+        if (st.n_tail >= 0 && il == hp.n_layer - 1) {
+            HIP_TRY(last_layer_tail(il, st));
+            tail_rows_ = st.n_tail;
+        } else if (st.engine) {
             HIP_TRY(launch_decode_engine(d_engine_layers_ + il, E, FF, d_engine_gran_, d_engine_epoch_, il, il == engine_probe_layer_ ? d_engine_probe_ : nullptr, stream_));
         } else {
             HIP_TRY(attn_output(il, st, ap));
@@ -1996,7 +2030,7 @@
     const HParams &hp = model->hp;
     const int E = hp.n_embd, V = hp.n_vocab;
     float *const xo = cur_T_ == 1 && n_out == 1 ? x_ : xo_;
-    if (xo != x_) HIP_TRY(launch_gather_rows_f32(x_, d_outrow_, n_out, E, xo_, stream_));
+    if (xo != x_ && tail_rows_ < 0) HIP_TRY(launch_gather_rows_f32(x_, d_outrow_, n_out, E, xo_, stream_));
     if (hp.encoder) {
         HIP_TRY(hipMemcpyAsync(d_embd_ + (size_t)out_base * E, xo, (size_t)n_out * E * 4, hipMemcpyDeviceToDevice, stream_));
         prof_mark("embd");
@@ -2128,6 +2162,7 @@
     if (attn_out_skip_step_) fused_skipped_steps++;
     bool graph_ok = cp.use_graphs && n == 1 && n_out == 1 && out_base == 0 && !profile_ && !debug_taps_ && !embeddings_enabled && moe_forced_T_ == 0 && !ub_embd_ && !attn_out_skip_step_ && !imx_on_;
     hipError_t e = hipSuccess;
+    tail_rows_ = -1;
     if (graph_ok) {
         int bucket = std::min((int)cp.n_ctx, (n_kv_ + 255) & ~255);
         chunk_cap_ = 0;
@@ -2143,7 +2178,7 @@
             e = hipStreamBeginCapture(stream_, hipStreamCaptureModeThreadLocal);
             if (e == hipSuccess) {
                 last_error.clear();
-                hipError_t e2 = run_layers(1, bucket > 0 ? bucket : std::min((int)cp.n_ctx, chunk_cap_ * 64));
+                hipError_t e2 = run_layers(1, bucket > 0 ? bucket : std::min((int)cp.n_ctx, chunk_cap_ * 64), 1);
                 if (e2 == hipSuccess) e2 = run_output(1, 0);
                 if (e2 == hipSuccess && cp.logits_to_host && !logits_on_host_) e2 = hipMemcpyAsync(h_logits_, d_logits_, (size_t)V * 4, hipMemcpyDeviceToHost, stream_);
                 if (e2 != hipSuccess) inner = last_error;
@@ -2170,7 +2205,7 @@
     if (!graph_ok) {
         prof_begin();
         chunk_cap_ = chunk_lmax_;
-        e = run_layers(n, n_kv_);
+        e = run_layers(n, n_kv_, n_out);
         if (e == hipSuccess) e = run_output(n_out, out_base);
         if (profiler_safe) (void)hipStreamSynchronize(stream_);
         if (e == hipSuccess && n_out > 0 && cp.logits_to_host && !embeddings_enabled && !logits_on_host_)
@@ -2693,7 +2728,7 @@
             if (hp.n_expert > 0) {
                 const int KU = hp.n_expert_used;
                 MMVQArgs a{}, d{};
-                if (!moe_ids_ || !moe_selected_desc(il, a, d)) continue;
+                if (!moe_ids_ || !moe_selected_desc(il, x_, a, d)) continue;
                 if (count) { std::vector<int32_t> ids((size_t)KU); for (int j = 0; j < KU; j++) ids[(size_t)j] = j; HIP_TRY(hipMemcpy(moe_ids_, ids.data(), ids.size() * 4, hipMemcpyHostToDevice)); }
                 HIP_TRY(launch_mmvq(a, stream_));
                 HIP_TRY(launch_mmvq(d, stream_));
diff --git a/cortex.llamacpp_amd/host/runtime.h b/cortex.llamacpp_amd/host/runtime.h
--- a/cortex.llamacpp_amd/host/runtime.h
+++ b/cortex.llamacpp_amd/host/runtime.h
@@ -92,6 +92,7 @@
 void set_moe_group_min(int tokens);
 void set_attn_store_fuse(bool on);
 void set_rope_fast(bool on);
+void set_last_layer_rows(int on);
 void set_decode_engine(int on);
 void set_decode_mega(bool on);
 
@@ -101,6 +102,7 @@
     int64_t qkv_attn_launches = 0;
     int64_t fused_skipped_steps = 0;
     int64_t mega_steps = 0;
+    int last_layer_rows() const { return tail_rows_; }
     Context(Model *m, const ContextParams &p);
     ~Context();
     bool init(std::string &err);
@@ -180,12 +182,15 @@
     size_t state_cell_bytes() const;
     struct Step {
         int T = 0, n_kv_max = 0;
+        int n_tail = -1;
         RopeArgs ra_step{};
         bool engine = false;
         bool tp = false;
         bool chunk_lists = false;
         int attn_mode = 2;
         bool rope_fast = true, fuse_down_env = true;
+        float *x = nullptr;
+        const float *att = nullptr;
         float *out = nullptr;
         const float *resid = nullptr;
     };
@@ -210,16 +215,17 @@
     hipError_t attn_output(int il, const Step &st, const AttnPlan &p);
     hipError_t ffn_block(int il, const Step &st);
     hipError_t ffn_moe(int il, const Step &st);
-    bool moe_selected_desc(int il, MMVQArgs &a, MMVQArgs &d) const;
-    hipError_t moe_grouped_one_launch(int il, int T);
-    hipError_t moe_grouped_per_expert(int il, int T, bool q80_any = false);
-    hipError_t moe_grouped_q80(int il, int T);
-    hipError_t moe_selected(int il, int T);
+    bool moe_selected_desc(int il, const float *x, MMVQArgs &a, MMVQArgs &d) const;
+    hipError_t moe_grouped_one_launch(int il, const Step &st);
+    hipError_t moe_grouped_per_expert(int il, const Step &st, bool q80_any = false);
+    hipError_t moe_grouped_q80(int il, const Step &st);
+    hipError_t moe_selected(int il, const Step &st);
     hipError_t ffn_dense_gate_up(int il, const Step &st, bool &quantised);
     hipError_t quantise_for_down(int il, int T, bool combined, bool planes_any_T);
     hipError_t ffn_down(int il, const Step &st, bool quantised, int *n_matvec = nullptr);
     hipError_t tap_layer(int il, int T);
-    hipError_t run_layers(int T, int n_kv_cap);
+    hipError_t run_layers(int T, int n_kv_cap, int n_out);
+    hipError_t last_layer_tail(int il, const Step &st);
     hipError_t run_layers_encoder(int T, int n_kv_cap);
     hipError_t run_output(int n_out, int out_base);
     hipError_t linear(const DevTensor &w, const ActQuant &aq, const float *x_f32, int K, int T, float *out, int ld_out,
@@ -252,6 +258,7 @@
 
     hipStream_t stream_ = nullptr;
     int cur_T_ = 0;
+    int tail_rows_ = -1;
     std::vector<void *> allocs_;
     std::vector<KVCell> cells_;
     int head_ = 0;
diff --git a/include/mi355_llama.h b/include/mi355_llama.h
--- a/include/mi355_llama.h
+++ b/include/mi355_llama.h
@@ -137,6 +137,7 @@
 MI355_API int64_t mi355_debug_engine_steps(const mi355_context *ctx);
 MI355_API int64_t mi355_debug_fused_skipped_steps(const mi355_context *ctx);
 MI355_API int64_t mi355_debug_qkv_attn_launches(const mi355_context *ctx);
+MI355_API int32_t mi355_debug_last_layer_rows(const mi355_context *ctx);
 MI355_API int64_t mi355_debug_qkv_attn_plan(int32_t type_q, int32_t type_k, int32_t type_v, int32_t type_o, int32_t n_embd, int32_t n_head, int32_t n_head_kv, int32_t head_dim,
                                             int32_t type_kv, int32_t n_kv, int32_t *slots_out);
 MI355_API void    mi355_set_embeddings(mi355_context *ctx, int32_t enabled);
```

Measured after the change: 677.4. Within noise of the previous version (-0.0%).
